# AO33/HiC_Genome_Assembler

Measured on AMD Instinct MI355X. Metric: Part1+Part2 wall-clock (s) and bins/s on N x N contact map, higher is better.
Workload: dtype f64

## Files before the change

### hic_genome_assembler_amd/_lib.py

```python
from __future__ import annotations

import ctypes
import os

import numpy as np

_HERE = os.path.dirname(os.path.abspath(__file__))
LIB_PATH = os.environ.get("HICMI_LIB") or os.path.join(_HERE, "libhicmi.so")
_lib = None

c_i64 = ctypes.c_int64
c_dbl = ctypes.c_double
_vp = ctypes.c_void_p
_M64 = (1 << 64) - 1

SIGNATURES = {
    "hicmi_abi_version": (ctypes.c_int, []),
    "hicmi_last_error": (ctypes.c_char_p, []),
    "hicmi_device_count": (ctypes.c_int, [ctypes.POINTER(ctypes.c_int)]),
    "hicmi_create": (ctypes.c_int, [ctypes.c_int, ctypes.POINTER(_vp)]),
    "hicmi_destroy": (ctypes.c_int, [_vp]),
    "hicmi_stream": (ctypes.c_int, [_vp, ctypes.POINTER(_vp)]),
    "hicmi_synchronize": (ctypes.c_int, [_vp]),
    "hicmi_set_contacts_host": (ctypes.c_int, [_vp, _vp, c_i64]),
    "hicmi_set_contacts_host_f32": (ctypes.c_int, [_vp, _vp, c_i64]),
    "hicmi_set_contacts_device": (ctypes.c_int, [_vp, _vp, c_i64, c_i64]),
    "hicmi_contacts_device": (ctypes.c_int, [_vp, ctypes.POINTER(_vp), ctypes.POINTER(c_i64), ctypes.POINTER(c_i64)]),
    "hicmi_load_hicpro_matrix": (ctypes.c_int, [ctypes.c_char_p, _vp, c_i64, _vp, ctypes.c_int, ctypes.POINTER(c_i64)]),
    "hicmi_row_sums": (ctypes.c_int, [_vp, _vp, _vp]),
    "hicmi_set_row_shard": (ctypes.c_int, [_vp, c_i64, c_i64]),
    "hicmi_set_row_sums": (ctypes.c_int, [_vp, _vp, _vp]),
    "hicmi_compact": (ctypes.c_int, [_vp, _vp, c_i64]),
    "hicmi_group_sums": (ctypes.c_int, [_vp, _vp, _vp, c_i64, c_i64, _vp, _vp]),
    "hicmi_upgma": (ctypes.c_int, [_vp, _vp, _vp]),
    "hicmi_rank_matrix": (ctypes.c_int, [_vp, _vp]),
    "hicmi_presort_state": (ctypes.c_int, [_vp, _vp, _vp]),
    "hicmi_get_rank_rows": (ctypes.c_int, [_vp, c_i64, c_i64, ctypes.c_int, _vp]),
    "hicmi_get_similarity_row": (ctypes.c_int, [_vp, c_i64, _vp]),
    "hicmi_cut_scan": (ctypes.c_int, [_vp, c_i64, c_i64, c_dbl, _vp, _vp]),
    "hicmi_filter_scan": (ctypes.c_int, [_vp, c_i64, c_i64, c_i64, c_i64, c_dbl, _vp, _vp]),
    "hicmi_first_pass_cuts": (ctypes.c_int, [_vp, c_i64, c_i64, c_dbl, _vp, c_i64, _vp, _vp, c_i64, _vp]),
    "hicmi_filter_cuts": (ctypes.c_int, [_vp, _vp, c_i64, c_dbl, _vp, c_i64, _vp, _vp]),
    "hicmi_first_pass_cuts_multi": (ctypes.c_int, [_vp, c_i64, _vp, _vp, c_dbl, _vp, c_i64, _vp, _vp, c_i64, _vp]),
    "hicmi_filter_cuts_multi": (ctypes.c_int, [_vp, c_i64, _vp, _vp, _vp, _vp, c_i64, _vp, _vp]),
    "hicmi_hypergeom_decide": (ctypes.c_int, [c_i64, c_i64, c_i64, c_i64, c_dbl]),
    "hicmi_hypergeom_sf": (c_dbl, [c_i64, c_i64, c_i64, c_i64]),
    "hicmi_selftest_division": (ctypes.c_int, [_vp, ctypes.c_uint64, c_i64, ctypes.POINTER(ctypes.c_uint64)]),
    "hicmi_label_linkage": (ctypes.c_int, [_vp, c_i64, _vp]),
    "hicmi_leaf_order": (ctypes.c_int, [_vp, c_i64, _vp]),
    "hicmi_get_raw_merges": (ctypes.c_int, [_vp, _vp]),
    "hicmi_nnchain_stats": (ctypes.c_int, [_vp, _vp]),
    "hicmi_p2_select": (ctypes.c_int, [_vp, _vp, c_i64]),
    "hicmi_p2_total": (ctypes.c_int, [_vp, ctypes.POINTER(c_dbl)]),
    "hicmi_p2_score": (ctypes.c_int, [_vp, _vp, c_i64, c_i64, c_dbl, _vp]),
    "hicmi_p2_score_exact": (ctypes.c_int, [_vp, _vp, c_i64, c_i64, c_dbl, _vp]),
    "hicmi_p2_layout": (ctypes.c_int, [_vp, _vp, _vp, c_i64]),
    "hicmi_p2_set_arrangement": (ctypes.c_int, [_vp, _vp, _vp, c_i64]),
    "hicmi_p2_arrangement_total": (ctypes.c_int, [_vp, ctypes.POINTER(c_dbl)]),
    "hicmi_p2_arrangement_score": (ctypes.c_int, [_vp, c_dbl, ctypes.POINTER(c_dbl)]),
    "hicmi_p2_score_insertions": (ctypes.c_int, [_vp, ctypes.c_int32, c_dbl, _vp]),
    "hicmi_p2_window_tables": (ctypes.c_int, [_vp, c_i64, _vp, c_i64, _vp, c_i64]),
    "hicmi_p2_score_window": (ctypes.c_int, [_vp, c_i64, c_i64, _vp]),
    "hicmi_p2_decide_window": (ctypes.c_int, [_vp, c_i64, c_i64, c_dbl, c_dbl, c_dbl, ctypes.POINTER(c_i64),
                                              ctypes.POINTER(c_dbl), ctypes.POINTER(c_dbl)]),
    "hicmi_p2_window_shortlist": (ctypes.c_int, [_vp, c_i64, c_i64, c_i64, c_dbl, c_dbl, c_dbl, c_i64, _vp, _vp, _vp]),
    "hicmi_p2_decide_insertion": (ctypes.c_int, [_vp, _vp, _vp, c_i64, ctypes.c_int32, ctypes.c_int32,
                                                 ctypes.POINTER(c_i64), ctypes.POINTER(ctypes.c_int32),
                                                 ctypes.POINTER(c_dbl)]),
    "hicmi_p2_insert_all": (ctypes.c_int, [_vp, _vp, _vp, c_i64, _vp, c_i64, ctypes.POINTER(c_dbl)]),
    "hicmi_scan_valid_pairs": (ctypes.c_int, [ctypes.c_char_p, ctypes.c_char_p, _vp, c_i64, _vp, _vp, c_i64, ctypes.c_int,
                                              ctypes.POINTER(c_i64), ctypes.POINTER(c_i64), ctypes.POINTER(_vp)]),
    "hicmi_scan_fetch": (ctypes.c_int, [_vp, _vp, _vp, _vp]),
    "hicmi_plot_percentiles": (ctypes.c_int, [_vp, ctypes.c_int, _vp, c_i64, _vp, c_i64, _vp]),
    "hicmi_plot_downsample": (ctypes.c_int, [_vp, ctypes.c_int, _vp, c_i64, c_i64, _vp]),
    "hicmi_p2_insert_all_multi": (ctypes.c_int, [c_i64, _vp, _vp, _vp, _vp, _vp, _vp, _vp]),
    "hicmi_p2_start_all": (ctypes.c_int, [c_i64] + [_vp] * 16),
    "hicmi_p2_scan_arranged": (ctypes.c_int, [_vp, _vp, _vp, c_i64, c_i64, _vp, c_i64, _vp, c_i64, ctypes.POINTER(c_dbl),
                                              ctypes.POINTER(c_dbl), ctypes.POINTER(c_i64)]),
    "hicmi_p2_support": (ctypes.c_int, [_vp, _vp, _vp, c_i64, c_dbl, _vp, _vp]),
    "hicmi_p2_support_multi": (ctypes.c_int, [c_i64, _vp, _vp, _vp, _vp, _vp, _vp, _vp]),
    "hicmi_p2_breaks": (ctypes.c_int, [_vp, _vp, _vp, c_i64, c_dbl, c_i64, _vp, _vp]),
    "hicmi_p2_breaks_multi": (ctypes.c_int, [c_i64, _vp, _vp, _vp, _vp, _vp, c_i64, _vp, _vp]),
    "hicmi_p2_scan_pass": (ctypes.c_int, [_vp, _vp, _vp, c_i64, c_i64, c_dbl, ctypes.POINTER(c_dbl), ctypes.POINTER(c_dbl),
                                          ctypes.POINTER(ctypes.c_int32)]),
    "hicmi_p2_scan_all": (ctypes.c_int, [_vp, _vp, _vp, c_i64, c_i64, c_dbl, ctypes.POINTER(c_dbl), ctypes.POINTER(c_dbl),
                          ctypes.POINTER(c_i64)]),
    "hicmi_hmm_load_obs": (ctypes.c_int, [_vp, _vp, c_i64, c_i64, c_i64]),
    "hicmi_hmm_set_obs": (ctypes.c_int, [_vp, _vp, c_i64, c_i64]),
    "hicmi_hmm_set_width": (ctypes.c_int, [_vp, c_i64]),
    "hicmi_hmm_get_obs": (ctypes.c_int, [_vp, c_i64, c_i64, _vp]),
    "hicmi_hmm_dist2": (ctypes.c_int, [_vp, _vp, c_i64, _vp]),
    "hicmi_hmm_col_stats": (ctypes.c_int, [_vp, _vp, _vp]),
    "hicmi_hmm_kmeans": (ctypes.c_int, [_vp, _vp, c_i64, c_dbl, _vp, _vp, ctypes.POINTER(c_dbl), ctypes.POINTER(c_i64)]),
    "hicmi_hmm_fit": (ctypes.c_int, [_vp, _vp, _vp, _vp, _vp, c_i64, c_dbl, _vp, ctypes.POINTER(c_i64)]),
    "hicmi_hmm_decode": (ctypes.c_int, [_vp, _vp, _vp, _vp, _vp, _vp]),
    "hicmi_hmm_load_obs_slot": (ctypes.c_int, [_vp, c_i64, _vp, c_i64, c_i64, c_i64]),
    "hicmi_hmm_use_obs": (ctypes.c_int, [_vp, c_i64]),
    "hicmi_hmm_dist2_multi": (ctypes.c_int, [_vp, c_i64, _vp, _vp, _vp, _vp, _vp]),
    "hicmi_hmm_kmeans_multi": (ctypes.c_int, [_vp, c_i64, _vp, _vp, _vp, _vp, _vp, _vp, _vp, _vp]),
    "hicmi_louvain_graph": (ctypes.c_int, [_vp, _vp, c_i64]),
    "hicmi_louvain_set_graph": (ctypes.c_int, [_vp, _vp, c_i64]),
    "hicmi_louvain_get_graph": (ctypes.c_int, [_vp, _vp, _vp, _vp]),
    "hicmi_louvain_level0": (ctypes.c_int, [_vp, c_i64, _vp, _vp, _vp, _vp, _vp, _vp]),
    "hicmi_louvain_induced": (ctypes.c_int, [_vp, _vp, c_i64, c_i64, _vp]),
    "hicmi_louvain_modularity": (ctypes.c_int, [_vp, _vp, c_i64, c_i64, _vp]),
    "hicmi_timing_reset": (ctypes.c_int, [_vp]),
    "hicmi_timing_enable": (ctypes.c_int, [_vp, ctypes.c_int]),
    "hicmi_timing_get": (ctypes.c_int, [_vp, ctypes.c_char_p, c_i64, _vp, _vp, _vp, c_i64, ctypes.POINTER(c_i64)]),
}


class HicmiError(RuntimeError):
    pass


def load():
    global _lib
    if _lib is not None:
        return _lib
    if not os.path.exists(LIB_PATH):
        raise HicmiError("libhicmi.so is not built (%s): run `make -C %s` - this package has no CPU fallback"
                         % (LIB_PATH, os.path.join(_HERE, "csrc")))
    try:
        import torch
    except ImportError:
        pass
    lib = ctypes.CDLL(LIB_PATH)
    for name, (res, args) in SIGNATURES.items():
        fn = getattr(lib, name)
        fn.restype = res
        fn.argtypes = args
    if lib.hicmi_abi_version() != 1:
        raise HicmiError("libhicmi ABI version mismatch")
    _lib = lib
    return lib


def _check(rc):
    if rc != 0:
        raise HicmiError("libhicmi error %d: %s" % (rc, load().hicmi_last_error().decode("utf-8", "replace")))


def _ptr(a):
    return None if a is None else a.ctypes.data_as(_vp)


def load_hicpro_matrix(path, bin_ids, threads: int = 0):
    ids = np.ascontiguousarray(bin_ids, dtype=np.int64)
    n = len(ids)
    out = np.empty((n, n), dtype=np.float64)
    edges = c_i64()
    _check(load().hicmi_load_hicpro_matrix(os.fsencode(path), _ptr(ids), n, _ptr(out), int(threads), ctypes.byref(edges)))
    return out, edges.value


def scan_valid_pairs(path, names, pairs, threads: int = 0):
    enc = [n.encode("utf-8") for n in names]
    blob = b"".join(enc)
    off = np.zeros(len(enc) + 1, np.int64)
    if enc:
        off[1:] = np.cumsum([len(e) for e in enc])
    pa = np.ascontiguousarray([p[0] for p in pairs], dtype=np.int32)
    pb = np.ascontiguousarray([p[1] for p in pairs], dtype=np.int32)
    n_hits, n_lines, handle = c_i64(), c_i64(), _vp()
    _check(load().hicmi_scan_valid_pairs(os.fsencode(path), blob, _ptr(off), len(enc), _ptr(pa), _ptr(pb), len(pa), int(threads),
                                         ctypes.byref(n_hits), ctypes.byref(n_lines), ctypes.byref(handle)))
    idx = np.empty(n_hits.value, np.int32)
    p1 = np.empty(n_hits.value, np.int64)
    p2 = np.empty(n_hits.value, np.int64)
    _check(load().hicmi_scan_fetch(handle, _ptr(idx), _ptr(p1), _ptr(p2)))
    return idx, p1, p2, n_lines.value


def hypergeom_sf(x, M, n, N) -> float:
    return float(load().hicmi_hypergeom_sf(int(x), int(M), int(n), int(N)))


def hypergeom_decide(x, M, n, N, psig) -> int:
    return int(load().hicmi_hypergeom_decide(int(x), int(M), int(n), int(N), float(psig)))


class Context:

    def __init__(self, device: int = 0):
        self._lib = load()
        h = _vp()
        _check(self._lib.hicmi_create(int(device), ctypes.byref(h)))
        self._h = h
        self.device = int(device)
        self.n = 0
        self._keepalive = None
        self._workers = []
        self._n_window_cand = 0
        self._lv_m = 0
        self.shard = (0, 1)

    def close(self):
        for w in getattr(self, "_workers", []):
            w.close()
        self._workers = []
        if getattr(self, "_h", None):
            self._lib.hicmi_destroy(self._h)
            self._h = None

    def workers(self, count: int):
        pool = getattr(self, "_workers", None)
        if pool is None:
            pool = self._workers = []
        ptr, n, ld = _vp(), c_i64(), c_i64()
        _check(self._lib.hicmi_contacts_device(self._h, ctypes.byref(ptr), ctypes.byref(n), ctypes.byref(ld)))
        while len(pool) < count:
            pool.append(Context(self.device))
        for w in pool[:count]:
            if getattr(w, "_shared_from", None) != (ptr.value, n.value, ld.value):
                w.set_contacts_device(ptr.value, n.value, ld.value, keepalive=self)
                w._shared_from = (ptr.value, n.value, ld.value)
        return pool[:count]

    def __del__(self):
        try:
            self.close()
        except Exception:
            pass

    def __enter__(self):
        return self

    def __exit__(self, *exc):
# ... 118 lines not shown

    def filter_cuts(self, cuts, psig):
        cuts = np.ascontiguousarray(cuts, dtype=np.int32)
        out = np.empty(self.n, np.int32)
        m, warned = c_i64(0), c_i64(0)
        _check(self._lib.hicmi_filter_cuts(self._h, _ptr(cuts), len(cuts), float(psig), _ptr(out), self.n,
                                           ctypes.byref(m), ctypes.byref(warned)))
        return [int(v) for v in out[:m.value]], int(warned.value)

    SCAN_MAX_SETS = 64

    def first_pass_cuts_multi(self, sets, psig):
        out = []
        n = self.n
        for c0 in range(0, len(sets), self.SCAN_MAX_SETS):
            part = sets[c0:c0 + self.SCAN_MAX_SETS]
            k = len(part)
            ms = np.array([int(a) for a, _b in part], np.int64)
            si = np.array([int(b) for _a, b in part], np.int64)
            cuts = np.empty((k, n), np.int32)
            mlog = np.empty((k, n, 2), np.int32)
            nc, nl = np.zeros(k, np.int64), np.zeros(k, np.int64)
            _check(self._lib.hicmi_first_pass_cuts_multi(self._h, k, _ptr(ms), _ptr(si), float(psig), _ptr(cuts), n,
                                                         _ptr(nc), _ptr(mlog), n, _ptr(nl)))
            out += [([int(v) for v in cuts[j, :nc[j]]], [(int(a), int(b)) for a, b in mlog[j, :nl[j]]]) for j in range(k)]
        return out

    def filter_cuts_multi(self, lists, psigs):
        out = []
        n = self.n
        for c0 in range(0, len(lists), self.SCAN_MAX_SETS):
            part = [np.asarray(v, dtype=np.int32) for v in lists[c0:c0 + self.SCAN_MAX_SETS]]
            k = len(part)
            off = np.zeros(k + 1, np.int64)
            off[1:] = np.cumsum([len(v) for v in part])
            cand = np.ascontiguousarray(np.concatenate(part) if off[-1] else np.zeros(1, np.int32), dtype=np.int32)
            ps = np.array([float(v) for v in psigs[c0:c0 + self.SCAN_MAX_SETS]], np.float64)
            kept = np.empty((k, n), np.int32)
            m, warned = np.zeros(k, np.int64), np.zeros(k, np.int64)
            _check(self._lib.hicmi_filter_cuts_multi(self._h, k, _ptr(off), _ptr(cand), _ptr(ps), _ptr(kept), n,
                                                     _ptr(m), _ptr(warned)))
            out += [([int(v) for v in kept[j, :m[j]]], int(warned[j])) for j in range(k)]
        return out

    def p2_select(self, sel):
        sel = np.ascontiguousarray(sel, dtype=np.int32)
        _check(self._lib.hicmi_p2_select(self._h, _ptr(sel), len(sel)))
        self._arr_sig = None

    def p2_total(self) -> float:
        t = c_dbl()
        _check(self._lib.hicmi_p2_total(self._h, ctypes.byref(t)))
        return t.value

    def p2_score(self, perms, total: float):
        perms = np.ascontiguousarray(perms, dtype=np.int32)
        if perms.ndim != 2:
            raise ValueError("perms must be (n_cand, n_used)")
        out = np.empty(perms.shape[0], np.float64)
        if perms.shape[0]:
            _check(self._lib.hicmi_p2_score(self._h, _ptr(perms), perms.shape[0], perms.shape[1], float(total), _ptr(out)))
        return out

    def p2_score_exact(self, perms, total: float):
        perms = np.ascontiguousarray(perms, dtype=np.int32)
        if perms.ndim != 2:
            raise ValueError("perms must be (n_cand, n_used)")
        out = np.empty(perms.shape[0], np.float64)
        if perms.shape[0]:
            _check(self._lib.hicmi_p2_score_exact(self._h, _ptr(perms), perms.shape[0], perms.shape[1], float(total),
                                                  _ptr(out)))
        return out

    def p2_layout(self, scaf_start, scaf_len):
        a = np.ascontiguousarray(scaf_start, dtype=np.int32)
        b = np.ascontiguousarray(scaf_len, dtype=np.int32)
        _check(self._lib.hicmi_p2_layout(self._h, _ptr(a), _ptr(b), len(a)))
        self._arr_sig = None

    def p2_set_arrangement(self, ids, rev):
        a = np.ascontiguousarray(ids, dtype=np.int32)
        b = np.ascontiguousarray(rev, dtype=np.uint8)
        sig = a.tobytes() + b.tobytes()
        if sig == getattr(self, "_arr_sig", None):
            return
        _check(self._lib.hicmi_p2_set_arrangement(self._h, _ptr(a), _ptr(b), len(a)))
        self._arr_len = len(a)
        self._arr_sig = sig

    def p2_arrangement_total(self) -> float:
        t = c_dbl()
        _check(self._lib.hicmi_p2_arrangement_total(self._h, ctypes.byref(t)))
        return t.value

    def p2_arrangement_score(self, total: float) -> float:
        t = c_dbl()
        _check(self._lib.hicmi_p2_arrangement_score(self._h, float(total), ctypes.byref(t)))
        return t.value

    def p2_score_insertions(self, new_id: int, total: float):
        out = np.empty(2 * (self._arr_len + 1), np.float64)
        _check(self._lib.hicmi_p2_score_insertions(self._h, int(new_id), float(total), _ptr(out)))
        return out

    def p2_window_tables(self, orders, orients):
        a = np.ascontiguousarray(orders, dtype=np.int8)
        b = np.ascontiguousarray(orients, dtype=np.uint8)
        _check(self._lib.hicmi_p2_window_tables(self._h, a.shape[1], _ptr(a), a.shape[0], _ptr(b), b.shape[0]))
        self._n_window_cand = a.shape[0] * b.shape[0]

    def p2_score_window(self, first: int, k: int):
        if not self._n_window_cand:
            raise HicmiError("p2_window_tables has not been called")
        out = np.empty(self._n_window_cand, np.float64)
        _check(self._lib.hicmi_p2_score_window(self._h, int(first), int(k), _ptr(out)))
        return out

    def p2_decide_window(self, first, k, total, floor, cur_fast):
        pick, best, pf = c_i64(), c_dbl(), c_dbl()
        _check(self._lib.hicmi_p2_decide_window(self._h, int(first), int(k), float(total), float(floor),
                                                float("nan") if cur_fast is None else float(cur_fast),
                                                ctypes.byref(pick), ctypes.byref(best), ctypes.byref(pf)))
        return pick.value, best.value, pf.value

    def p2_window_shortlist(self, first, count, k, total, floor, cur_fast=None, cap=4096):
        n_near = np.zeros(int(count), np.int64)
        idx = np.zeros((int(count), int(cap)), np.int64)
        fast = np.zeros((int(count), int(cap)), np.float64)
        _check(self._lib.hicmi_p2_window_shortlist(self._h, int(first), int(count), int(k), float(total), float(floor),
                                                   float("nan") if cur_fast is None else float(cur_fast), int(cap),
                                                   _ptr(n_near), _ptr(idx), _ptr(fast)))
        return [None if m > cap else (idx[w, :m].copy(), fast[w, :m].copy()) for w, m in enumerate(n_near.tolist())]

    def p2_decide_insertion(self, ids, rev, new_id, new_rev_now):
        a = np.ascontiguousarray(ids, dtype=np.int32)
        b = np.ascontiguousarray(rev, dtype=np.uint8)
        gap, r, best = c_i64(), ctypes.c_int32(), c_dbl()
        _check(self._lib.hicmi_p2_decide_insertion(self._h, _ptr(a), _ptr(b), len(a), int(new_id), int(new_rev_now),
                                                   ctypes.byref(gap), ctypes.byref(r), ctypes.byref(best)))
        self._arr_sig = a.tobytes() + b.tobytes()
        self._arr_len = len(a)
        return gap.value, r.value, best.value

    def p2_insert_all(self, ids, rev, new_ids):
        s0, k = len(ids), len(new_ids)
        a = np.zeros(s0 + k, np.int32); a[:s0] = ids
        b = np.zeros(s0 + k, np.uint8); b[:s0] = rev
        nw = np.ascontiguousarray(new_ids, dtype=np.int32)
        best = c_dbl()
        _check(self._lib.hicmi_p2_insert_all(self._h, _ptr(a), _ptr(b), s0, _ptr(nw), k, ctypes.byref(best)))
        self._arr_sig = None
        return a, b, best.value

    @staticmethod
    def p2_insert_all_multi(jobs):
        n = len(jobs)
        if n == 0:
            return []
        lib = jobs[0][0]._lib
        keep, a_l, b_l, nw_l = [], [], [], []
        for ctx, ids, rev, new_ids in jobs:
            s0, k = len(ids), len(new_ids)
            a = np.zeros(s0 + k, np.int32); a[:s0] = ids
            b = np.zeros(s0 + k, np.uint8); b[:s0] = rev
            a_l.append(a); b_l.append(b); nw_l.append(np.ascontiguousarray(new_ids, dtype=np.int32))
        handles = (ctypes.c_void_p * n)(*[j[0]._h for j in jobs])
        pa = (ctypes.c_void_p * n)(*[x.ctypes.data for x in a_l])
        pb = (ctypes.c_void_p * n)(*[x.ctypes.data for x in b_l])
        pn = (ctypes.c_void_p * n)(*[x.ctypes.data for x in nw_l])
        s0s = (c_i64 * n)(*[len(j[1]) for j in jobs])
        ks = (c_i64 * n)(*[len(j[3]) for j in jobs])
        best = (c_dbl * n)()
        _check(lib.hicmi_p2_insert_all_multi(n, handles, pa, pb, s0s, pn, ks, best))
        for ctx, _i, _r, _n in jobs:
            ctx._arr_sig = None
        return [(a_l[j], b_l[j], best[j]) for j in range(n)]

    @staticmethod
    def p2_start_all(jobs, tables):
        n = len(jobs)
        if n == 0:
            return []
        lib = jobs[0][0]._lib
        i32 = lambda col: np.ascontiguousarray(np.concatenate([np.asarray(j[col], dtype=np.int32) for j in jobs]), dtype=np.int32)
        sel, st, ln, ids = i32(1), i32(2), i32(3), i32(4)
        n_sel = (c_i64 * n)(*[len(j[1]) for j in jobs])
        n_scaf = (c_i64 * n)(*[len(j[2]) for j in jobs])
        ks = (c_i64 * n)(*[len(j[4]) for j in jobs])
        keep = {k: (np.ascontiguousarray(o, dtype=np.int8), np.ascontiguousarray(r, dtype=np.uint8)) for k, (o, r) in tables.items()}
        po = (ctypes.c_void_p * 9)(*[keep[k][0].ctypes.data if k in keep else None for k in range(9)])
        pr = (ctypes.c_void_p * 9)(*[keep[k][1].ctypes.data if k in keep else None for k in range(9)])
        no = (c_i64 * 9)(*[keep[k][0].shape[0] if k in keep else 0 for k in range(9)])
        nr = (c_i64 * 9)(*[keep[k][1].shape[0] if k in keep else 0 for k in range(9)])
        handles = (ctypes.c_void_p * n)(*[j[0]._h for j in jobs])
        total, pick, cost, status = (c_dbl * n)(), (c_i64 * n)(), (c_dbl * n)(), (ctypes.c_int32 * n)()
        _check(lib.hicmi_p2_start_all(n, handles, _ptr(sel), n_sel, _ptr(st), _ptr(ln), n_scaf, _ptr(ids), ks, po, no, pr, nr,
                                      total, pick, cost, status))
        for j, job in enumerate(jobs):
            ctx, k = job[0], len(job[4])
            ctx._arr_sig, ctx._arr_len = None, k
            if status[j] != 1:
                ctx._n_window_cand = keep[k][0].shape[0] * keep[k][1].shape[0]
        return [(total[j], int(pick[j]), cost[j], int(status[j])) for j in range(n)]

    def p2_scan_arranged(self, ids, rev, k, orders, orients, best):
        a = np.ascontiguousarray(ids, dtype=np.int32).copy()
        b = np.ascontiguousarray(rev, dtype=np.uint8).copy()
        o = np.ascontiguousarray(orders, dtype=np.int8)
        r = np.ascontiguousarray(orients, dtype=np.uint8)
        bst, total, rounds = c_dbl(float(best)), c_dbl(), c_i64()
        _check(self._lib.hicmi_p2_scan_arranged(self._h, _ptr(a), _ptr(b), len(a), int(k), _ptr(o), o.shape[0], _ptr(r), r.shape[0],
                                                ctypes.byref(total), ctypes.byref(bst), ctypes.byref(rounds)))
        self._arr_sig = None
        self._n_window_cand = o.shape[0] * r.shape[0]
        return a, b, bst.value, int(rounds.value), total.value

    def p2_support(self, ids, rev, total: float):
        a = np.ascontiguousarray(ids, dtype=np.int32)
        b = np.ascontiguousarray(rev, dtype=np.uint8)
        S = len(a)
        table, best = np.empty((S, S, 2), np.float64), np.empty((S, 2), np.int32)
        _check(self._lib.hicmi_p2_support(self._h, _ptr(a), _ptr(b), S, float(total), _ptr(table), _ptr(best)))
        self._arr_sig = a.tobytes() + b.tobytes()
        self._arr_len = S
        return table, best

    @staticmethod
    def p2_support_multi(jobs):
        n = len(jobs)
        if n == 0:
            return []
        lib = jobs[0][0]._lib
        a_l = [np.ascontiguousarray(j[1], dtype=np.int32) for j in jobs]
        b_l = [np.ascontiguousarray(j[2], dtype=np.uint8) for j in jobs]
        t_l = [np.empty((len(a), len(a), 2), np.float64) for a in a_l]
        o_l = [np.empty((len(a), 2), np.int32) for a in a_l]
        handles = (ctypes.c_void_p * n)(*[j[0]._h for j in jobs])
        pa, pb, pt, po = ((ctypes.c_void_p * n)(*[x.ctypes.data for x in arrs]) for arrs in (a_l, b_l, t_l, o_l))
        sizes = (c_i64 * n)(*[len(a) for a in a_l])
        totals = (c_dbl * n)(*[float(j[3]) for j in jobs])
        _check(lib.hicmi_p2_support_multi(n, handles, pa, pb, sizes, totals, pt, po))
        for (ctx, _i, _r, _t), a, b in zip(jobs, a_l, b_l):
            ctx._arr_sig = a.tobytes() + b.tobytes()
            ctx._arr_len = len(a)
        return list(zip(t_l, o_l))

    def p2_breaks(self, ids, rev, lengths, total: float, min_piece: int = 1):
        return Context.p2_breaks_multi([(self, ids, rev, lengths, total)], min_piece, single=True)[0]

    @staticmethod
    def p2_breaks_multi(jobs, min_piece: int = 1, single=False):
        n = len(jobs)
        if n == 0:
            return []
        lib = jobs[0][0]._lib
        a_l = [np.ascontiguousarray(j[1], dtype=np.int32) for j in jobs]
        b_l = [np.ascontiguousarray(j[2], dtype=np.uint8) for j in jobs]
        t_l = [np.empty((sum(max(int(ln) - 1, 0) for ln in j[3]), 8), np.float64) for j in jobs]
        o_l = [np.empty((len(a), 2), np.int32) for a in a_l]
        if single:
            _check(lib.hicmi_p2_breaks(jobs[0][0]._h, _ptr(a_l[0]), _ptr(b_l[0]), len(a_l[0]), float(jobs[0][4]), int(min_piece),
                                       t_l[0].ctypes.data, _ptr(o_l[0])))
        else:
            handles = (ctypes.c_void_p * n)(*[j[0]._h for j in jobs])
            pa, pb, pt, po = ((ctypes.c_void_p * n)(*[x.ctypes.data for x in arrs]) for arrs in (a_l, b_l, t_l, o_l))
            sizes = (c_i64 * n)(*[len(a) for a in a_l])
            totals = (c_dbl * n)(*[float(j[4]) for j in jobs])
            _check(lib.hicmi_p2_breaks_multi(n, handles, pa, pb, sizes, totals, int(min_piece), pt, po))
        for j, a, b in zip(jobs, a_l, b_l):
            j[0]._arr_sig = a.tobytes() + b.tobytes()
            j[0]._arr_len = len(a)
        return list(zip(t_l, o_l))

    def p2_scan_pass(self, ids, rev, k, total, best, cur_fast):
        a = np.ascontiguousarray(ids, dtype=np.int32).copy()
        b = np.ascontiguousarray(rev, dtype=np.uint8).copy()
        bst = c_dbl(float(best))
        cf = c_dbl(float("nan") if cur_fast is None else float(cur_fast))
        imp = ctypes.c_int32()
        _check(self._lib.hicmi_p2_scan_pass(self._h, _ptr(a), _ptr(b), len(a), int(k), float(total), ctypes.byref(bst),
                                            ctypes.byref(cf), ctypes.byref(imp)))
        self._arr_sig = None
        return a, b, bst.value, cf.value, bool(imp.value)

    def p2_scan_all(self, ids, rev, k, total, best, cur_fast):
        a = np.ascontiguousarray(ids, dtype=np.int32).copy()
        b = np.ascontiguousarray(rev, dtype=np.uint8).copy()
        bst = c_dbl(float(best))
        cf = c_dbl(float("nan") if cur_fast is None else float(cur_fast))
        rounds = c_i64()
        _check(self._lib.hicmi_p2_scan_all(self._h, _ptr(a), _ptr(b), len(a), int(k), float(total), ctypes.byref(bst),
                                           ctypes.byref(cf), ctypes.byref(rounds)))
        self._arr_sig = None
        return a, b, bst.value, cf.value, int(rounds.value)

    def plot_percentiles(self, kind, order, q):
        qa = np.ascontiguousarray(q, dtype=np.float64)
        out = np.empty(len(qa), np.float64)
        if order is None:
            n_sel, optr, keep = self.n, None, None
        else:
            keep = np.ascontiguousarray(order, dtype=np.int32)
            n_sel, optr = len(keep), _ptr(keep)
        _check(self._lib.hicmi_plot_percentiles(self._h, int(kind), optr, n_sel, _ptr(qa), len(qa), _ptr(out)))
        return out

# ... 232 lines not shown
```

### hic_genome_assembler_amd/csrc/api.hip

```cpp
#include <hip/hip_runtime.h>

#include <algorithm>
#include <cmath>
#include <cstdarg>
#include <climits>
#include <cstdio>
#include <cstdlib>
#include <cstring>
#include <numeric>
#include <string>
#include <unordered_map>
#include <functional>
#include <chrono>
#include <vector>

#include "../../include/hicmi.h"
#include "hicmi_internal.h"
#include "hyper.h"

using namespace hicmi;

static thread_local std::string g_err;

static int fail(int code, const char* fmt, ...)
{
    char buf[512];
    va_list ap;
    va_start(ap, fmt);
    vsnprintf(buf, sizeof(buf), fmt, ap);
    va_end(ap);
    g_err = buf;
    return code;
}

namespace hicmi { int set_error(int code, const char* msg) { return fail(code, "%s", msg); } }

#define HIPCHK(expr)                                                                              \
    do {                                                                                          \
        hipError_t _e = (expr);                                                                   \
        if (_e != hipSuccess) return fail(HICMI_EHIP, "%s: %s", #expr, hipGetErrorString(_e));     \
    } while (0)

enum Family { F_ROW_SUMS, F_BUILD_W, F_NNCHAIN, F_SORT, F_RANK_INVERT, F_CUT_COUNT, F_HYPER_FLAGS, F_P2_SELECT,
              F_P2_TOTAL, F_P2_SCORE, F_P2_EXACT, F_P2_INSERT, F_P2_WINDOW_G, F_P2_WINDOW_DELTA, F_PLOT, F_PRESORT, F_RANK_RELABEL,
              F_RANK_TIED, F_P2_WINDOW_FLOPS, F_COUNT };
static const char* kFamilyNames[F_COUNT] = {"row_sums", "build_w", "nnchain", "sort_rows", "rank_invert",
                                            "cut_count", "hyper_flags", "p2_select", "p2_total", "p2_score",
                                            "p2_score_exact", "p2_score_insert", "p2_window_G", "p2_window_delta", "plot",
                                            "presort_rows", "rank_relabel", "rank_rows_tied",
                                            "p2_window_G_flops"};

constexpr int kBaseSlabs = 256;

struct TimedRegion { int fam; hipEvent_t a, b; };

struct hicmi_ctx {
    int device = 0;
    hipStream_t stream = nullptr;
    int probed_xcc = 0;
    int64_t n = 0, ldc = 0;
    double* dC = nullptr;
    bool own_c = false;
    double *d_np = nullptr, *d_seq = nullptr;
    bool have_sums = false;
    int64_t shard_first = 0, shard_stride = 1;
    double *dW = nullptr, *dW2 = nullptr; int64_t ldw = 0; int64_t w_rows = 0;
    int *d_size = nullptr, *d_chain = nullptr, *d_status = nullptr;
    double* d_zraw = nullptr;
    std::vector<double> zraw;
    int32_t* d_order = nullptr;
    uint16_t *dR = nullptr, *dRank = nullptr; int64_t ldr = 0; int64_t r_rows = 0;
    void* d_sort_scratch = nullptr; size_t sort_scratch_cap = 0;
    bool have_rank = false;
    hipStream_t stream2 = nullptr; hipEvent_t ev_fork = nullptr, ev_join = nullptr;
    uint16_t* dRankS = nullptr; int64_t rank_s_rows = 0;
    int32_t* d_ident = nullptr; int64_t ident_cap = 0;
    unsigned char* d_ties = nullptr; int64_t ties_cap = 0;
    uint16_t* d_tie_bits = nullptr; int64_t tie_bits_rows = 0, ld_bits = 0;
    int32_t* d_row_list = nullptr; int64_t row_list_cap = 0;
    int64_t scan_first_batch = 0, scan_last_improved = 0;
    int64_t presort_tied_rows = 0;
    int presort_used = 0;
    int64_t presort_n = 0;
    bool presort_dealt = false;
    int32_t* d_x = nullptr; uint8_t* d_sig = nullptr; int64_t x_cap = 0;
    unsigned char* d_scan_multi = nullptr; size_t scan_multi_bytes = 0;
    int64_t cached_start = -1;
    double* d_tmp = nullptr; int64_t tmp_cap = 0;
    double* dM2 = nullptr; int64_t n2 = 0, ld2 = 0, m2_cap = 0;
    int32_t* d_sel = nullptr; int64_t sel_cap = 0;
    double* d_H = nullptr; int64_t h_cap = 0;
    int32_t* d_perms = nullptr; int64_t perms_cap = 0;
    double* d_scores = nullptr; int64_t scores_cap = 0;
    double* d_partial = nullptr; int64_t partial_cap = 0;
    double* d_T = nullptr; int64_t t_cap = 0;
    int32_t *d_scaf_start = nullptr, *d_scaf_len = nullptr; int64_t scaf_cap = 0, n_scaf = 0;
    std::vector<int32_t> h_scaf_start, h_scaf_len;
    int32_t* d_arr_packed = nullptr; int64_t arr_cap = 0;
    std::vector<int32_t> h_arr_packed;
    std::vector<int32_t> h_arr_id, h_arr_pos; std::vector<uint8_t> h_arr_rev;
    int32_t* d_pos2sel = nullptr; int64_t pos_cap = 0; int64_t n_arr = 0;
    int8_t* d_orders = nullptr; uint8_t* d_orients = nullptr; int64_t ord_cap = 0, ori_cap = 0;
    int tab_k = 0; int64_t n_orders = 0, n_orients = 0;
    std::vector<int8_t> h_orders; std::vector<uint8_t> h_orients;
    std::vector<int32_t> h_pos2sel;
    uint64_t arr_version = 0;
    uint64_t cur_lit_version = ~0ull; double cur_lit_total = 0.0, cur_lit_value = 0.0;
    double cache_total = 0.0; bool cache_valid = false;
    std::unordered_map<std::string, double> exact_cache;
    double* d_G = nullptr; int64_t g_cap = 0;
    double* d_delta = nullptr; int64_t delta_cap = 0;
    WindowBatchEntry* d_wb = nullptr; int64_t wb_cap = 0;
    int near_min_k = 7;
    unsigned char* d_wnear = nullptr; int64_t wnear_cap = 0;
    int32_t* d_arr_packed2 = nullptr; int64_t arr2_cap = 0;
    int32_t* d_pos2sel2 = nullptr; int64_t pos2_cap = 0;
    double* d_ins_T = nullptr; int64_t ins_t_cap = 0;
    double* d_ins_partial = nullptr; int64_t ins_partial_cap = 0;
    unsigned char* d_ins_blob = nullptr; int64_t ins_blob_cap = 0;
    InsStep* d_ins_steps = nullptr; int64_t ins_steps_cap = 0;
    SupRec* d_sup_recs = nullptr; int64_t sup_recs_cap = 0;
    BrkRec* d_brk_recs = nullptr; int64_t brk_recs_cap = 0;
    int32_t* d_gs_lists = nullptr; int64_t gs_lists_cap = 0;
    double* d_gs_sums = nullptr; int64_t gs_sums_cap = 0;
    struct HmmSlot { double* d_x = nullptr; int64_t cap = 0, T = 0, ld = 0, D = 0; };
    HmmSlot hslot[HICMI_HMM_MAX_SLOTS]; int hcur = 0;
    double* d_hx = nullptr; int64_t hmm_T = 0, hmm_ld = 0, hmm_D = 0;
    unsigned char* d_hmulti = nullptr; int64_t hmulti_cap = 0;
    int32_t* d_horder = nullptr; int64_t horder_cap = 0;
    double* d_hwork = nullptr; int64_t hwork_cap = 0;
    int32_t* d_hlab = nullptr; int64_t hlab_cap = 0;
    uint8_t* d_hbt = nullptr; int64_t hbt_cap = 0;
    double* d_hpart = nullptr; int64_t hpart_cap = 0;
    double* d_hsmall = nullptr; int64_t hsmall_cap = 0;
    double* d_hhist = nullptr; int64_t hhist_cap = 0;
    int* d_hst = nullptr; int64_t hst_cap = 0;
    double* d_lvA = nullptr; int64_t lvA_cap = 0; int64_t lv_m = 0;
    double* d_lvvec = nullptr; int64_t lvvec_cap = 0;
    int32_t* d_lvrows = nullptr; int64_t lvrows_cap = 0;
    unsigned char* d_lvwork = nullptr; int64_t lvwork_cap = 0;
    int32_t* d_plot_order = nullptr; int64_t plot_order_cap = 0;
    unsigned char* d_plot_work = nullptr; int64_t plot_work_cap = 0;
    double* d_plot_img = nullptr; int64_t plot_img_cap = 0;
    char* pin_up = nullptr; size_t pin_up_cap = 0, pin_up_off = 0;
    char* pin_down = nullptr; size_t pin_down_cap = 0;

    int timing = 0;
    std::vector<TimedRegion> regions;
    std::vector<hipEvent_t> pool;
    double ms[F_COUNT] = {0}; int64_t launches[F_COUNT] = {0}; double bytes[F_COUNT] = {0};
    double nn_scans = 0, nn_scan_cols = 0, nn_cache_hits = 0, nn_merges = 0; int64_t nn_retries = 0;
};

namespace {
hipError_t sync_stream(hicmi_ctx* c);

struct Timed {
    hicmi_ctx* c; int fam; hipEvent_t a = nullptr, b = nullptr; hipStream_t st;
    Timed(hicmi_ctx* ctx, int f, double algo_bytes, hipStream_t on_stream = nullptr) : c(ctx), fam(f), st(on_stream ? on_stream : ctx->stream)
    {
        c->launches[f]++; c->bytes[f] += algo_bytes;
        if (!on()) return;
        a = grab(); b = grab();
        hipEventRecord(a, st);
    }
    bool on() const { return c->timing == 1 || (c->timing == 2 && (fam <= F_RANK_INVERT || fam >= F_PRESORT)); }
    ~Timed()
    {
        if (!on()) return;
        hipEventRecord(b, st);
        c->regions.push_back({fam, a, b});
    }
    hipEvent_t grab()
    {
        if (!c->pool.empty()) { hipEvent_t e = c->pool.back(); c->pool.pop_back(); return e; }
        hipEvent_t e; hipEventCreate(&e); return e;
    }
};

int resolve_timing(hicmi_ctx* c)
{
    if (c->regions.empty()) return HICMI_OK;
    HIPCHK(sync_stream(c));
    if (c->stream2) HIPCHK(hipStreamSynchronize(c->stream2));
    for (auto& r : c->regions) {
        float ms = 0.f;
        if (hipEventElapsedTime(&ms, r.a, r.b) == hipSuccess) c->ms[r.fam] += ms;
        c->pool.push_back(r.a); c->pool.push_back(r.b);
    }
    c->regions.clear();
    return HICMI_OK;
}


hipError_t sync_stream(hicmi_ctx* c)
{
    hipError_t e = hipStreamSynchronize(c->stream);
    c->pin_up_off = 0;
    return e;
}

int upload(hicmi_ctx* c, void* dst, const void* src, size_t bytes)
{
    if (bytes == 0) return HICMI_OK;
    const size_t need = (bytes + 63) & ~(size_t)63;
    if (c->pin_up_off + need > c->pin_up_cap) {
        HIPCHK(sync_stream(c));
        if (need > c->pin_up_cap) {
            if (c->pin_up) (void)hipHostFree(c->pin_up);
            c->pin_up = nullptr; c->pin_up_cap = 0;
            size_t cap = std::max<size_t>(need * 2, (size_t)1 << 20);
            HIPCHK(hipHostMalloc((void**)&c->pin_up, cap, hipHostMallocDefault));
            c->pin_up_cap = cap;
        }
    }
    char* slot = c->pin_up + c->pin_up_off;
    memcpy(slot, src, bytes);
    c->pin_up_off += need;
    HIPCHK(hipMemcpyAsync(dst, slot, bytes, hipMemcpyHostToDevice, c->stream));
    return HICMI_OK;
}

int ensure_pin_down(hicmi_ctx* c, size_t bytes)
{
    if (bytes > c->pin_down_cap) {
        if (c->pin_down) (void)hipHostFree(c->pin_down);
        c->pin_down = nullptr; c->pin_down_cap = 0;
        size_t cap = std::max<size_t>(bytes * 2, (size_t)1 << 20);
        HIPCHK(hipHostMalloc((void**)&c->pin_down, cap, hipHostMallocDefault));
        c->pin_down_cap = cap;
    }
    return HICMI_OK;
}

int download(hicmi_ctx* c, void* dst, const void* src, size_t bytes)
{
    if (bytes == 0) { HIPCHK(sync_stream(c)); return HICMI_OK; }
    int rc_pin = ensure_pin_down(c, bytes);
    if (rc_pin) return rc_pin;
    HIPCHK(hipMemcpyAsync(c->pin_down, src, bytes, hipMemcpyDeviceToHost, c->stream));
    HIPCHK(sync_stream(c));
    memcpy(dst, c->pin_down, bytes);
    return HICMI_OK;
}

template <typename T>
int ensure(T*& p, int64_t& cap, int64_t need)
{
    if (need <= cap && p) return HICMI_OK;
    if (p) { (void)hipFree(p); p = nullptr; cap = 0; }
    if (need <= 0) need = 1;
    hipError_t e = hipMalloc((void**)&p, (size_t)need * sizeof(T));
    if (e != hipSuccess) { p = nullptr; return fail(HICMI_ENOMEM, "hipMalloc(%lld bytes): %s", (long long)(need * (int64_t)sizeof(T)), hipGetErrorString(e)); }
    cap = need;
    return HICMI_OK;
}

void free_dev(void* p) { if (p) (void)hipFree(p); }

void drop_matrix_state(hicmi_ctx* c)
{
    if (c->own_c) free_dev(c->dC);
    c->dC = nullptr; c->own_c = false; c->n = 0; c->ldc = 0;
    free_dev(c->d_np); free_dev(c->d_seq); c->d_np = c->d_seq = nullptr; c->have_sums = false;
    c->have_rank = false; c->cached_start = -1; c->n2 = 0;
    if (c->presort_n && c->stream2) (void)hipStreamSynchronize(c->stream2);
    c->presort_n = 0;
}

int alloc_sums(hicmi_ctx* c)
{
    HIPCHK(hipMalloc((void**)&c->d_np, sizeof(double) * (size_t)std::max<int64_t>(c->n, 1)));
    HIPCHK(hipMalloc((void**)&c->d_seq, sizeof(double) * (size_t)std::max<int64_t>(c->n, 1)));
// ... 1696 lines not shown
    int rc = window_near_enqueue(c, first0, count, k, total, floor, cur_fast, cap, p);
    if (rc) return rc;
    return window_near_collect(c, p, n_near, near, near_fast);
}

const int64_t kNearCap = 4096;

int check_window_call(hicmi_ctx* c, int64_t first, int64_t k)
{
    const int64_t S = (int64_t)c->h_arr_id.size();
    if (c->n_arr < 1 || S < 1) return fail(HICMI_EINVAL, "hicmi_p2_set_arrangement has not run");
    if (k != c->tab_k || c->h_orders.empty()) return fail(HICMI_EINVAL, "hicmi_p2_window_tables has not been called for k = %lld", (long long)k);
    if (first < 0 || first + k > S) return fail(HICMI_EINVAL, "window out of range");
    for (int64_t j = 0; j < k; j++) if (c->h_orders[(size_t)j] != j) return fail(HICMI_EINVAL, "orders[0] must be the identity");
    return HICMI_OK;
}
}

int hicmi_p2_decide_window(hicmi_ctx* c, int64_t first, int64_t k, double total, double floor, double cur_fast,
                           int64_t* pick_out, double* best_out, double* pick_fast_out)
{
    if (!c || !pick_out || !best_out || !pick_fast_out) return fail(HICMI_EINVAL, "NULL argument");
    int rc = check_window_call(c, first, k);
    if (rc) return rc;
    use_total(c, total);
    if (k >= c->near_min_k) {
        std::vector<int64_t> n_near; std::vector<std::vector<int64_t>> near; std::vector<std::vector<double>> near_fast;
        rc = window_near_batch(c, first, 1, k, total, floor, cur_fast, kNearCap, n_near, near, near_fast);
        if (rc) return rc;
        if (n_near[0] <= kNearCap)
            return decide_from_near(c, first, k, total, floor, cur_fast, window_c0(c, first, k), near[0], near_fast[0],
                                    pick_out, best_out, pick_fast_out);
    }
    std::vector<double> delta((size_t)(c->n_orders * c->n_orients));
    rc = window_batch(c, first, 1, k, delta.data());
    if (rc) return rc;
    return decide_from_delta(c, first, k, total, floor, cur_fast, delta.data(), pick_out, best_out, pick_fast_out);
}

int hicmi_p2_window_shortlist(hicmi_ctx* c, int64_t first, int64_t count, int64_t k, double total, double floor,
                              double cur_fast, int64_t cap, int64_t* n_near_out, int64_t* idx_out, double* fast_out)
{
    if (!c || !n_near_out || !idx_out || !fast_out || count < 1) return fail(HICMI_EINVAL, "bad arguments");
    int rc = check_window_call(c, first, k);
    if (rc) return rc;
    std::vector<int64_t> n_near; std::vector<std::vector<int64_t>> near; std::vector<std::vector<double>> near_fast;
    rc = window_near_batch(c, first, count, k, total, floor, cur_fast, cap, n_near, near, near_fast);
    if (rc) return rc;
    for (int64_t w = 0; w < count; w++) {
        n_near_out[w] = n_near[(size_t)w];
        for (size_t q = 0; q < near[(size_t)w].size(); q++) {
            idx_out[w * cap + (int64_t)q] = near[(size_t)w][q];
            fast_out[w * cap + (int64_t)q] = near_fast[(size_t)w][q];
        }
    }
    return HICMI_OK;
}

int hicmi_p2_decide_insertion(hicmi_ctx* c, const int32_t* ids, const uint8_t* rev, int64_t S, int32_t new_id,
                              int32_t new_rev_now, int64_t* gap_out, int32_t* rev_out, double* best_out)
{
    if (!c || !ids || !rev || !gap_out || !rev_out || !best_out || S < 1) return fail(HICMI_EINVAL, "bad arguments");
    if (c->n_scaf < 1) return fail(HICMI_EINVAL, "hicmi_p2_layout has not run");
    if (new_id < 0 || new_id >= c->n_scaf) return fail(HICMI_EINVAL, "new scaffold out of range");
    *gap_out = -1; *rev_out = 0; *best_out = 0.0;
    std::vector<int32_t> ids2(ids, ids + S); ids2.push_back(new_id);
    std::vector<uint8_t> rev2(rev, rev + S); rev2.push_back(new_rev_now ? 1 : 0);
    int rc = hicmi_p2_set_arrangement(c, ids2.data(), rev2.data(), S + 1);
    if (rc) return rc;
    double total = 0.0;
    rc = hicmi_p2_arrangement_total(c, &total);
    if (rc) return rc;
    use_total(c, total);
    rc = hicmi_p2_set_arrangement(c, ids, rev, S);
    if (rc) return rc;
    const int64_t gaps = S + 1;
    std::vector<double> by_gap_rev((size_t)(2 * gaps));
    rc = hicmi_p2_score_insertions(c, new_id, total, by_gap_rev.data());
    if (rc) return rc;
    std::vector<double> fast((size_t)(2 * gaps));
    std::vector<int32_t> tag_rev((size_t)(2 * gaps));
    int32_t o = new_rev_now ? 1 : 0;
    for (int64_t i = 0; i < gaps; i++) {
        tag_rev[(size_t)(2 * i)] = o; tag_rev[(size_t)(2 * i + 1)] = o ^ 1;
        fast[(size_t)(2 * i)] = by_gap_rev[(size_t)(2 * i + o)];
        fast[(size_t)(2 * i + 1)] = by_gap_rev[(size_t)(2 * i + (o ^ 1))];
        o ^= 1;
    }
    std::vector<int64_t> near;
    short_list(fast, 0.0, near);
    if (near.empty()) return HICMI_OK;
    const int32_t st = c->h_scaf_start[(size_t)new_id], ln = c->h_scaf_len[(size_t)new_id];
    std::vector<std::vector<int32_t>> rows(near.size());
    for (size_t q = 0; q < near.size(); q++) {
        const int64_t g = near[q] / 2;
        const int32_t r = tag_rev[(size_t)near[q]];
        const int P = c->h_arr_pos[(size_t)g];
        std::vector<int32_t>& row = rows[q];
        row.reserve((size_t)(c->n_arr + ln));
        row.insert(row.end(), c->h_pos2sel.begin(), c->h_pos2sel.begin() + P);
        if (r) for (int32_t e = 0; e < ln; e++) row.push_back(st + ln - 1 - e);
        else   for (int32_t e = 0; e < ln; e++) row.push_back(st + e);
        row.insert(row.end(), c->h_pos2sel.begin() + P, c->h_pos2sel.end());
    }
    std::vector<double> lit;
    rc = literal_scores(c, rows, total, lit);
    if (rc) return rc;
    double best = 0.0; int64_t pick = -1;
    for (size_t q = 0; q < near.size(); q++) if (lit[q] > best) { best = lit[q]; pick = near[q]; }
    if (pick >= 0) { *gap_out = pick / 2; *rev_out = tag_rev[(size_t)pick]; *best_out = best; }
    return HICMI_OK;
}


namespace {
void apply_insertion(int32_t* ids, uint8_t* rev, int64_t& S, int64_t gap, int32_t new_id, int32_t r)
{
    for (int64_t j = S; j > gap; j--) { ids[j] = ids[j - 1]; rev[j] = rev[j - 1]; }
    ids[gap] = new_id; rev[gap] = (uint8_t)(r ? 1 : 0);
    S++;
}

struct InsJob {
    hicmi_ctx* c; int32_t* ids; uint8_t* rev; int64_t S; const int32_t* new_ids; int64_t n_new;
    int64_t t = 0; double best = 0.0; bool device_ok = true;
};

int queue_insertions(hicmi_ctx* lead, const std::vector<InsJob*>& jobs)
{
    const int nj = (int)jobs.size();
    if (nj == 0) return HICMI_OK;
    const int NB = kBaseSlabs;
    static const int max_c = getenv("HICMI_P2_INS_MAXC") ? atoi(getenv("HICMI_P2_INS_MAXC")) : INS_MAXC;
    int64_t steps_max = 0;
    std::vector<size_t> blob_off((size_t)nj);
    size_t blob_bytes = 0;
    for (int j = 0; j < nj; j++) {
        InsJob& job = *jobs[(size_t)j];
        hicmi_ctx* c = job.c;
        int rc = hicmi_p2_set_arrangement(c, job.ids, job.rev, job.S);
        if (rc) return rc;
        if (c != lead) HIPCHK(sync_stream(c));
        const int64_t n_steps = job.n_new - job.t;
        int64_t n_max = c->n_arr;
        for (int64_t t = 0; t < n_steps; t++) n_max += c->h_scaf_len[(size_t)job.new_ids[job.t + t]];
        if (n_max * (int64_t)sizeof(int32_t) > 160 * 1024) return fail(HICMI_EUNSUPPORTED, "candidate longer than 40960 bins");
        const int64_t S_max = job.S + n_steps;
        rc = ensure(c->d_arr_packed2, c->arr2_cap, 3 * std::max<int64_t>(S_max, c->n_scaf) + 2);
        if (rc) return rc;
        rc = ensure(c->d_pos2sel2, c->pos2_cap, c->n2);
        if (rc) return rc;
        rc = ensure(c->d_ins_T, c->ins_t_cap, (1 + 2 * (int64_t)INS_MAXC) * n_max);
        if (rc) return rc;
        rc = ensure(c->d_ins_partial, c->ins_partial_cap, NB + n_max + 2 * (S_max + 1));
        if (rc) return rc;
        steps_max = std::max(steps_max, n_steps);
        blob_off[(size_t)j] = blob_bytes;
        blob_bytes += (sizeof(InsState) + sizeof(InsLog) * (size_t)n_steps + 15) & ~(size_t)15;
    }
    HIPCHK(hipSetDevice(lead->device));
    int rc = ensure(lead->d_ins_blob, lead->ins_blob_cap, (int64_t)blob_bytes);
    if (rc) return rc;
    rc = ensure(lead->d_ins_steps, lead->ins_steps_cap, steps_max * nj);
    if (rc) return rc;
    std::vector<InsStep> table((size_t)(steps_max * nj));
    std::vector<int> max_n_used((size_t)steps_max, 0), max_S((size_t)steps_max, 0), max_n_arr((size_t)steps_max, 0);
    double algo = 0.0;
    for (int j = 0; j < nj; j++) {
        InsJob& job = *jobs[(size_t)j];
        hicmi_ctx* c = job.c;
        const int64_t n_steps = job.n_new - job.t;
        int64_t n_max = c->n_arr;
        for (int64_t t = 0; t < n_steps; t++) n_max += c->h_scaf_len[(size_t)job.new_ids[job.t + t]];
        InsState* st = reinterpret_cast<InsState*>(lead->d_ins_blob + blob_off[(size_t)j]);
        InsLog* log = reinterpret_cast<InsLog*>(lead->d_ins_blob + blob_off[(size_t)j] + sizeof(InsState));
        int32_t* packed[2] = {c->d_arr_packed, c->d_arr_packed2};
        int32_t* pos2sel[2] = {c->d_pos2sel, c->d_pos2sel2};
        int64_t n_arr = c->n_arr;
        for (int64_t t = 0; t < steps_max; t++) {
            InsStep& d = table[(size_t)(t * nj + j)];
            memset(&d, 0, sizeof(d));
            d.st = st;
            if (t >= n_steps) continue;
            const int cur = (int)(t & 1), nxt = cur ^ 1;
            const int32_t nid = job.new_ids[job.t + t];
            const int L = c->h_scaf_len[(size_t)nid];
            d.M2 = c->dM2; d.H = c->d_H; d.ld2 = c->ld2;
            d.pos_cur = pos2sel[cur]; d.pos_nxt = pos2sel[nxt]; d.packed_cur = packed[cur]; d.packed_nxt = packed[nxt];
            d.T_total = c->d_ins_T; d.T_cand = c->d_ins_T + n_max; d.work = c->d_ins_T + (1 + (int64_t)INS_MAXC) * n_max;
            d.partial = c->d_ins_partial; d.log = log + t;
            d.n_arr = (int32_t)n_arr; d.S = (int32_t)(job.S + t); d.L = L; d.new_start = c->h_scaf_start[(size_t)nid];
            d.new_id = nid; d.active = 1; d.step = (int32_t)t; d.last = t == n_steps - 1;
            max_n_used[(size_t)t] = std::max(max_n_used[(size_t)t], (int)(n_arr + L));
            max_S[(size_t)t] = std::max(max_S[(size_t)t], d.S);
            max_n_arr[(size_t)t] = std::max(max_n_arr[(size_t)t], (int)n_arr);
            const double nn = (double)n_arr, Ld = (double)L, sd = (double)d.S;
            algo += 8.0 * (0.5 * nn * (nn - 1.0) + nn * nn + 2.0 * (sd + 1.0) * Ld * nn) + 4.0 * (nn + Ld) * (nn + Ld);
            n_arr += L;
        }
    }
    rc = upload(lead, lead->d_ins_steps, table.data(), sizeof(InsStep) * table.size());
    if (rc) return rc;
    {
        Timed timed(lead, F_P2_INSERT, algo);
        launch_insb_reset(lead->d_ins_steps, nj, lead->stream);
        for (int64_t t = 0; t < steps_max; t++) {
            const InsStep* st_t = lead->d_ins_steps + t * nj;
            const int nu = max_n_used[(size_t)t];
            launch_insb_fast(st_t, nj, max_S[(size_t)t], max_n_arr[(size_t)t], NB, lead->stream);
            launch_insb_shortlist(st_t, nj, max_S[(size_t)t], max_n_arr[(size_t)t], NB, kNearTop, max_c, lead->stream);
            launch_insb_diag_cand(st_t, nj, nu, lead->stream);
            launch_insb_cost(st_t, nj, nu, lead->stream);
            launch_insb_apply(st_t, nj, nu, lead->stream);
        }
    }
    HIPCHK(hipGetLastError());
    std::vector<unsigned char> blob(blob_bytes);
    rc = download(lead, blob.data(), lead->d_ins_blob, blob_bytes);
    if (rc) return rc;
    if (getenv("HICMI_PART2_PROFILE")) {
        int64_t hist[5] = {0, 0, 0, 0, 0}, all_direct = 0;
        for (int64_t t = 0; t < steps_max; t++) {
            int mx = -1, ran = 0;
            for (int j = 0; j < nj; j++) {
                if (t >= jobs[(size_t)j]->n_new - jobs[(size_t)j]->t) continue;
                const InsState* hs = reinterpret_cast<const InsState*>(blob.data() + blob_off[(size_t)j]);
                if (hs->fail >= 0 && t >= hs->fail) continue;
                const InsLog* hl = reinterpret_cast<const InsLog*>(blob.data() + blob_off[(size_t)j] + sizeof(InsState));
                const int ns = hl[t].n_short;
                hist[ns < 0 ? 0 : (ns > 3 ? 4 : ns + 1)]++;
                mx = std::max(mx, ns);
                ran++;
            }
            if (ran && mx < 0) all_direct++;
        }
        fprintf(stderr, "[hicmi] insertion short lists: direct %lld, literal with 0:%lld 1:%lld 2:%lld 3+:%lld candidates; "
                        "lock steps without any literal pass: %lld of %lld\n",
                (long long)hist[0], (long long)hist[1], (long long)hist[2], (long long)hist[3], (long long)hist[4],
                (long long)all_direct, (long long)steps_max);
    }
    for (int j = 0; j < nj; j++) {
        InsJob& job = *jobs[(size_t)j];
        const int64_t n_steps = job.n_new - job.t;
        const InsState* hst = reinterpret_cast<const InsState*>(blob.data() + blob_off[(size_t)j]);
        const InsLog* hlog = reinterpret_cast<const InsLog*>(blob.data() + blob_off[(size_t)j] + sizeof(InsState));
        const int64_t done = hst->fail >= 0 ? std::min<int64_t>(hst->fail, n_steps) : n_steps;
        for (int64_t t = 0; t < done; t++) {
            if (hlog[t].gap < 0 || hlog[t].gap > job.S) return fail(HICMI_ESTATE, "insertion log out of range");
            apply_insertion(job.ids, job.rev, job.S, hlog[t].gap, job.new_ids[job.t + t], hlog[t].rev);
            job.best = hlog[t].best;
        }
        job.t += done;
        hicmi_ctx* c = job.c;
        c->n_arr = 0; c->h_arr_id.clear(); c->h_arr_rev.clear(); c->h_arr_pos.clear(); c->h_pos2sel.clear();
    }
    return HICMI_OK;
}

int check_insert_job(const InsJob& job, int64_t S0)
{
    hicmi_ctx* c = job.c;
    if (!c || !job.ids || !job.rev || !job.new_ids || S0 < 1 || job.n_new < 1) return fail(HICMI_EINVAL, "bad arguments");
    if (c->n_scaf < 1) return fail(HICMI_EINVAL, "hicmi_p2_layout has not run");
    std::vector<uint8_t> used((size_t)c->n_scaf, 0);
    for (int64_t j = 0; j < S0 + job.n_new; j++) {
        const int32_t v = j < S0 ? job.ids[j] : job.new_ids[j - S0];
        if (v < 0 || v >= c->n_scaf || used[(size_t)v]) return fail(HICMI_EINVAL, "scaffolds must be distinct members of the layout");
        used[(size_t)v] = 1;
    }
    return HICMI_OK;
}

int host_insertion_step(InsJob& job)
{
    int64_t gap = -1; int32_t r = 0;
    int rc = hicmi_p2_decide_insertion(job.c, job.ids, job.rev, job.S, job.new_ids[job.t], 0, &gap, &r, &job.best);
    if (rc) return rc;
    if (gap < 0) { gap = 0; r = 0; job.best = 0.0; }
    apply_insertion(job.ids, job.rev, job.S, gap, job.new_ids[job.t], r);
    job.t++;
    return HICMI_OK;
}

int run_insert_jobs(std::vector<InsJob>& all)
{
    static const bool host_only = getenv("HICMI_P2_HOST_INSERT") != nullptr;
    for (InsJob& job : all) {
        int rc = check_insert_job(job, job.S);
        if (rc) return rc;
        if (job.S + job.n_new + 1 > 8192) job.device_ok = false;
    }
    while (true) {
        std::vector<InsJob*> todo;
        for (InsJob& job : all) if (job.t < job.n_new && job.device_ok && !host_only) todo.push_back(&job);
        if (!todo.empty()) {
            int rc = queue_insertions(todo[0]->c, todo);
            if (rc) return rc;
        }
        bool pending = false;
        for (InsJob& job : all) {
            if (job.t >= job.n_new) continue;
            do {
                int rc = host_insertion_step(job);
                if (rc) return rc;
            } while (job.t < job.n_new && (host_only || !job.device_ok));
            if (job.t < job.n_new) pending = true;
        }
        if (!pending) break;
    }
    return HICMI_OK;
}
}

int hicmi_p2_insert_all(hicmi_ctx* c, int32_t* ids, uint8_t* rev, int64_t S0, const int32_t* new_ids, int64_t n_new,
                        double* best_out)
{
    if (!c || !best_out) return fail(HICMI_EINVAL, "bad arguments");
    std::vector<InsJob> jobs(1);
    jobs[0].c = c; jobs[0].ids = ids; jobs[0].rev = rev; jobs[0].S = S0; jobs[0].new_ids = new_ids; jobs[0].n_new = n_new;
    int rc = run_insert_jobs(jobs);
    if (rc) return rc;
    *best_out = jobs[0].best;
    return HICMI_OK;
}

int hicmi_p2_insert_all_multi(int64_t n_jobs, hicmi_ctx* const* ctxs, int32_t* const* ids, uint8_t* const* rev,
                              const int64_t* S0, const int32_t* const* new_ids, const int64_t* n_new, double* best_out)
{
    if (n_jobs < 1 || !ctxs || !ids || !rev || !S0 || !new_ids || !n_new || !best_out) return fail(HICMI_EINVAL, "bad arguments");
    std::vector<InsJob> jobs((size_t)n_jobs);
    for (int64_t j = 0; j < n_jobs; j++) {
        InsJob& job = jobs[(size_t)j];
        job.c = ctxs[j]; job.ids = ids[j]; job.rev = rev[j]; job.S = S0[j]; job.new_ids = new_ids[j]; job.n_new = n_new[j];
        if (!job.c || job.c->device != ctxs[0]->device) return fail(HICMI_EINVAL, "contexts must share one device");
        for (int64_t q = 0; q < j; q++) if (ctxs[q] == ctxs[j]) return fail(HICMI_EINVAL, "one context per chromosome");
    }
    int rc = run_insert_jobs(jobs);
    if (rc) return rc;
    for (int64_t j = 0; j < n_jobs; j++) best_out[j] = jobs[(size_t)j].best;
    return HICMI_OK;
}

int hicmi_p2_support_multi(int64_t n_jobs, hicmi_ctx* const* ctxs, const int32_t* const* ids, const uint8_t* const* rev,
                           const int64_t* S, const double* totals, double* const* scores_out, int32_t* const* best_out)
{
    if (n_jobs < 1 || !ctxs || !ids || !rev || !S || !totals || !scores_out || !best_out) return fail(HICMI_EINVAL, "bad arguments");
    hicmi_ctx* lead = ctxs[0];
    const int NB = SUP_BASE_SLABS;
    std::vector<size_t> out_off((size_t)n_jobs, 0);
    std::vector<uint8_t> run((size_t)n_jobs, 0);
    size_t blob_bytes = 0;
    int64_t n_rec = 0;
    int max_S = 1, max_n = 1;
    for (int64_t j = 0; j < n_jobs; j++) {
        hicmi_ctx* c = ctxs[j];
        if (!c || !lead || c->device != lead->device) return fail(HICMI_EINVAL, "contexts must share one device");
        for (int64_t q = 0; q < j; q++) if (ctxs[q] == c) return fail(HICMI_EINVAL, "one context per chromosome");
        if (!ids[j] || !rev[j] || !scores_out[j] || !best_out[j] || S[j] < 1) return fail(HICMI_EINVAL, "bad arguments");
        if (S[j] > SUP_MAX_S) return fail(HICMI_EUNSUPPORTED, "more than %d scaffolds in one chromosome", SUP_MAX_S);
        int rc = hicmi_p2_set_arrangement(c, ids[j], rev[j], S[j]);
        if (rc) return rc;
        if (c != lead) HIPCHK(sync_stream(c));
        if (c->n_arr * (int64_t)sizeof(int32_t) > 160 * 1024) return fail(HICMI_EUNSUPPORTED, "candidate longer than 40960 bins");
        for (int64_t i = 0; i < 2 * S[j] * S[j]; i++) scores_out[j][i] = 0.0;
        for (int64_t i = 0; i < S[j]; i++) { best_out[j][2 * i] = -1; best_out[j][2 * i + 1] = 0; }
        if (c->n_arr < 2 || !(totals[j] > 0.0)) continue;
        run[(size_t)j] = 1;
        rc = ensure(c->d_ins_partial, c->ins_partial_cap, S[j] * (NB + c->n_arr + 2 * S[j]));
        if (rc) return rc;
        out_off[(size_t)j] = blob_bytes;
        blob_bytes += ((size_t)(2 * S[j] * S[j]) * sizeof(double) + (size_t)(2 * S[j]) * sizeof(int32_t) + 15) & ~(size_t)15;
        n_rec += S[j];
        max_S = std::max(max_S, (int)S[j]);
        max_n = std::max(max_n, (int)c->n_arr);
    }
    if (n_rec == 0) return HICMI_OK;
    HIPCHK(hipSetDevice(lead->device));
    int rc = ensure(lead->d_ins_blob, lead->ins_blob_cap, (int64_t)blob_bytes);
    if (rc) return rc;
    rc = ensure(lead->d_sup_recs, lead->sup_recs_cap, n_rec);
    if (rc) return rc;
    std::vector<SupRec> recs;
    recs.reserve((size_t)n_rec);
    double algo = 0.0;
    for (int64_t j = 0; j < n_jobs; j++) {
        if (!run[(size_t)j]) continue;
        hicmi_ctx* c = ctxs[j];
        const int64_t Sj = S[j], n = c->n_arr;
        double* d_scores = reinterpret_cast<double*>(lead->d_ins_blob + out_off[(size_t)j]);
        int32_t* d_best = reinterpret_cast<int32_t*>(d_scores + 2 * Sj * Sj);
        for (int64_t k = 0; k < Sj; k++) {
            SupRec d;
            memset(&d, 0, sizeof(d));
            const int32_t sid = ids[j][k];
            d.M2 = c->dM2; d.H = c->d_H; d.ld2 = c->ld2;
            d.pos = c->d_pos2sel; d.arr_pos = c->d_arr_packed + Sj;
            d.partial = c->d_ins_partial + k * (NB + n + 2 * Sj);
            d.scores = d_scores + 2 * Sj * k; d.best = d_best + 2 * k;
            d.total = totals[j];
            d.n = (int32_t)n; d.S = (int32_t)Sj; d.j = (int32_t)k;
            d.start = c->h_scaf_start[(size_t)sid]; d.L = c->h_scaf_len[(size_t)sid]; d.cur_rev = rev[j][k] ? 1 : 0;
            recs.push_back(d);
            const double nn = (double)(n - d.L);
            algo += 8.0 * (0.5 * nn * nn + nn * nn + 2.0 * (double)Sj * (double)d.L * nn);
        }
    }
    rc = upload(lead, lead->d_sup_recs, recs.data(), sizeof(SupRec) * recs.size());
    if (rc) return rc;
    {
        Timed timed(lead, F_P2_INSERT, algo);
        launch_sup(lead->d_sup_recs, (int)n_rec, max_S, max_n, kNearTop, lead->stream);
    }
    HIPCHK(hipGetLastError());
    std::vector<unsigned char> blob(blob_bytes);
    rc = download(lead, blob.data(), lead->d_ins_blob, blob_bytes);
    if (rc) return rc;
    for (int64_t j = 0; j < n_jobs; j++) {
        if (!run[(size_t)j]) continue;
        const size_t nd = (size_t)(2 * S[j] * S[j]);
        memcpy(scores_out[j], blob.data() + out_off[(size_t)j], nd * sizeof(double));
        memcpy(best_out[j], blob.data() + out_off[(size_t)j] + nd * sizeof(double), (size_t)(2 * S[j]) * sizeof(int32_t));
    }
    return HICMI_OK;
}

int hicmi_p2_support(hicmi_ctx* c, const int32_t* ids, const uint8_t* rev, int64_t S, double total, double* scores_out,
                     int32_t* best_out)
{
    return hicmi_p2_support_multi(1, &c, &ids, &rev, &S, &total, &scores_out, &best_out);
}

int hicmi_p2_breaks_multi(int64_t n_jobs, hicmi_ctx* const* ctxs, const int32_t* const* ids, const uint8_t* const* rev,
                          const int64_t* S, const double* totals, int64_t min_piece, double* const* scores_out,
                          int32_t* const* best_out)
{
    if (n_jobs < 1 || !ctxs || !ids || !rev || !S || !totals || !scores_out || !best_out || min_piece < 1)
        return fail(HICMI_EINVAL, "bad arguments");
    hicmi_ctx* lead = ctxs[0];
    const int NB = BRK_BASE_SLABS;
    std::vector<size_t> out_off((size_t)n_jobs, 0);
    std::vector<int64_t> n_scores((size_t)n_jobs, 0);
    std::vector<uint8_t> run((size_t)n_jobs, 0);
    size_t blob_bytes = 0;
    int64_t n_rec = 0;
    for (int64_t j = 0; j < n_jobs; j++) {
        hicmi_ctx* c = ctxs[j];
        if (!c || !lead || c->device != lead->device) return fail(HICMI_EINVAL, "contexts must share one device");
        for (int64_t q = 0; q < j; q++) if (ctxs[q] == c) return fail(HICMI_EINVAL, "one context per chromosome");
        if (!ids[j] || !rev[j] || !scores_out[j] || !best_out[j] || S[j] < 1) return fail(HICMI_EINVAL, "bad arguments");
        int rc = hicmi_p2_set_arrangement(c, ids[j], rev[j], S[j]);
        if (rc) return rc;
        if (c != lead) HIPCHK(sync_stream(c));
        if (c->n_arr * (int64_t)sizeof(int32_t) > 160 * 1024) return fail(HICMI_EUNSUPPORTED, "candidate longer than 40960 bins");
        int64_t cand = 0, scratch = NB, multi = 0;
        for (int64_t k = 0; k < S[j]; k++) {
            const int64_t L = c->h_scaf_len[(size_t)ids[j][k]];
            if (L < 2) continue;
            cand += 8 * (L - 1); scratch += L * L + 3 * (L - 1); multi++;
        }
        n_scores[(size_t)j] = cand;
        for (int64_t i = 0; i < cand; i++) scores_out[j][i] = 0.0;
        for (int64_t i = 0; i < S[j]; i++) { best_out[j][2 * i] = -1; best_out[j][2 * i + 1] = 0; }
        if (c->n_arr < 2 || !(totals[j] > 0.0) || multi == 0) continue;
        run[(size_t)j] = 1;
        rc = ensure(c->d_ins_partial, c->ins_partial_cap, scratch);
        if (rc) return rc;
        out_off[(size_t)j] = blob_bytes;
        blob_bytes += ((size_t)cand * sizeof(double) + (size_t)(2 * S[j]) * sizeof(int32_t) + 15) & ~(size_t)15;
        n_rec += multi;
    }
    if (n_rec == 0) return HICMI_OK;
    HIPCHK(hipSetDevice(lead->device));
    int rc = ensure(lead->d_ins_blob, lead->ins_blob_cap, (int64_t)blob_bytes);
    if (rc) return rc;
    rc = ensure(lead->d_brk_recs, lead->brk_recs_cap, n_rec);
// ... 1024 lines not shown
```

### hic_genome_assembler_amd/csrc/hicmi_internal.h

```cpp
#pragma once
#include <hip/hip_runtime.h>
#include <stdint.h>

#include <atomic>
#include <functional>

namespace hicmi {

inline void ensure_dynamic_lds(const void* func, std::atomic<int>& have, size_t bytes)
{
    if ((int)bytes > have.load(std::memory_order_relaxed)) {
        (void)hipFuncSetAttribute(func, hipFuncAttributeMaxDynamicSharedMemorySize, (int)bytes);
        have.store((int)bytes, std::memory_order_relaxed);
    }
}

static constexpr int SERIAL_BATCH = 16;

__device__ __forceinline__ double serial_sum_lds(const double* t, int from, int to, double acc)
{
    constexpr int B = SERIAL_BATCH;
    int i = from;
    if (i + B <= to) {
        double a[B];
// ... 111 lines not shown
                        int own_first, int own_step, hipStream_t s);

struct ScanState {
    int done;
    int mode;
    int start, cut, n_rows, recount;
    long long M;
    double psig;
    int min_size, stop_ind, loop_count, n_cuts, n_log, scans;
    int MD, n_alt, alt_off, f_i, f_keep_from, f_noise, f_round, f_max_rounds, f_warned;
    int pad;
    unsigned long long bytes;
};
static constexpr int SCAN_MAX_SETS = 64;
void launch_first_pass_multi_pairs(const uint16_t* rank, int64_t ldr, int n, int n_sets, ScanState* st, int32_t* x, uint8_t* sig,
                                   double psig0, int share, int32_t* cuts, int32_t* mlog, int log_cap, int pairs, hipStream_t s);
void launch_filter_multi_pairs(const uint16_t* rank, int64_t ldr, int n, int max_rows, int n_sets, ScanState* st, int32_t* x,
                               uint8_t* sig, double psig0, int share, int32_t* alt, uint8_t* filt, uint8_t* prev,
                               int32_t* seg, int32_t* seg_x, int pairs, hipStream_t s);

#if defined(__HIPCC__)
template <int M>
__device__ __forceinline__ uint32_t xor_lane(uint32_t v, int lane)
{
    if constexpr (M == 1) return (uint32_t)__builtin_amdgcn_mov_dpp((int)v, 0xB1, 0xf, 0xf, true);
    else if constexpr (M == 2) return (uint32_t)__builtin_amdgcn_mov_dpp((int)v, 0x4E, 0xf, 0xf, true);
    else if constexpr (M == 4) {
        const int t = __builtin_amdgcn_mov_dpp((int)v, 0x141, 0xf, 0xf, true);
        return (uint32_t)__builtin_amdgcn_mov_dpp(t, 0x1B, 0xf, 0xf, true);
    } else if constexpr (M == 8) {
        const int t = __builtin_amdgcn_mov_dpp((int)v, 0x140, 0xf, 0xf, true);
        return (uint32_t)__builtin_amdgcn_mov_dpp(t, 0x141, 0xf, 0xf, true);
    } else if constexpr (M == 16) {
        const auto r = __builtin_amdgcn_permlane16_swap(v, v, false, false);
        return (lane & 16) ? r[0] : r[1];
    } else {
        static_assert(M == 32, "xor_lane: M must be 1, 2, 4, 8, 16 or 32");
        const auto r = __builtin_amdgcn_permlane32_swap(v, v, false, false);
        return (lane & 32) ? r[0] : r[1];
    }
}
#endif

int  sort_padded_size(int n);
int  sort_workgroups(int n);
size_t sort_scratch_bytes(int n);
struct SortExtras {
    const int32_t* row_list = nullptr; int n_list = 0;
    uint8_t* tie_flag = nullptr; unsigned* tie_count = nullptr; unsigned tie_limit = 0;
    uint16_t* tie_bits = nullptr; int64_t ld_bits = 0;
    int max_workgroups = 0;
    int avoid_xcc = -1; unsigned* row_counter = nullptr;
};
static constexpr int GETREG_XCC_ID = 20 | (0 << 6) | (3 << 11);
int nnchain_local_xcc(const NNChainOptions& o, int n);
void launch_sort_rows(const double* C, int64_t ldc, const int32_t* order, const int32_t* inv, const double* np_sum,
                      const double* seq_sum, int n, void* scratch, uint16_t* R, int64_t ldr, int row_first, int row_stride,
                      hipStream_t s, const SortExtras& x = SortExtras());
void launch_rank_rows_tied(const uint16_t* R_storage, const uint16_t* tie_bits, int64_t ld_bits, const int32_t* order,
                           const int32_t* inv, int n, const int32_t* row_list, int n_list, uint16_t* rank, int64_t ldr,
                           hipStream_t s, int32_t* done = nullptr);
void launch_rank_relabel(const uint16_t* rank_storage, uint16_t* rank, int64_t ldr, int n, const int32_t* order, int row_first,
                         int row_stride, hipStream_t s);
size_t sort_radix_scratch_bytes(int n);
void launch_rank_rows_radix(const double* C, int64_t ldc, const int32_t* order, const int32_t* inv, const double* np_sum,
                            const double* seq_sum, int n, void* scratch, uint16_t* rank, int64_t ldr, int row_first,
                            int row_stride, hipStream_t s);
void launch_rank_invert(const uint16_t* R, uint16_t* rank, int64_t ldr, int n, int row_first, int row_stride, hipStream_t s,
                        const int32_t* row_list = nullptr, int n_list = 0);
void launch_similarity_row(const double* C, int64_t ldc, const int32_t* order, const double* np_sum,
                           const double* seq_sum, int n, int row, double* out, hipStream_t s);

void launch_p2_select(const double* C, int64_t ldc, const int32_t* sel, int n, double* M2, int64_t ld2, hipStream_t s);
void launch_p2_total(const double* M2, int64_t ld2, int n, double* T, double* total, hipStream_t s);
void launch_p2_score_exact(const double* M2, int64_t ld2, const int32_t* perms, int n_cand, int n_used, double total,
                           double* T, double* work, double* scores, hipStream_t s);
void launch_p2_score(const double* M2, int64_t ld2, const int32_t* perms, int n_cand, int n_used, const double* H,
                     double inv_total_unused, double total, double* scores, hipStream_t s);

void launch_p2_total_perm(const double* M2, int64_t ld2, const int32_t* d_perm, int n, double* T, double* total,
                          hipStream_t s);

struct WindowDesc {
    int32_t start[8];
    int32_t len[8];
    int32_t off[8];
    uint8_t rev[8];
};
void launch_arr_materialize(const int32_t* packed, int S, const int32_t* scaf_start, const int32_t* scaf_len, int n_arr,
                            int32_t* pos2sel, hipStream_t s);
void launch_p2_base_partial(const double* M2, int64_t ld2, const int32_t* pos2sel, int n_arr, const double* H, int n_tot,
                            int n_blocks, double* out, hipStream_t s);
void launch_p2_insert_delta(const double* M2, int64_t ld2, const int32_t* pos2sel, int n_arr, const int32_t* arr_pos,
                            int S, int new_start, int L, const double* H, int n_base_blocks, double* out, hipStream_t s);
struct WindowBatchEntry {
    WindowDesc w;
    int32_t p0, m;
    int64_t g_off;
    int32_t c0, pad;
};
void launch_p2_window_batch(const double* M2, int64_t ld2, const int32_t* pos2sel, int n, int k,
                            const WindowBatchEntry* wb, int n_win, int max_m, const int8_t* orders, const uint8_t* orients,
                            int n_ord, int n_ori, const double* H, double* G_all, double* delta_all, hipStream_t s);


int64_t window_table_doubles(int k);
void launch_p2_window_tables(const double* M2, int64_t ld2, const int32_t* pos2sel, int n, int k,
                             const WindowBatchEntry* wb, const WindowBatchEntry* h_wb, int n_win, int max_m, const int8_t* orders, const uint8_t* orients,
                             int n_ord, int n_ori, const double* H, double* tables, double* delta_all, hipStream_t s);
struct NearEntry { int32_t cand, pad; double fast; };
int window_near_blocks(int n_ord);
void launch_p2_window_near(const double* M2, int64_t ld2, const int32_t* pos2sel, int n, int k,
                           const WindowBatchEntry* wb, const WindowBatchEntry* h_wb, int n_win, int max_m, const int8_t* orders,
                           const uint8_t* orients, int n_ord, int n_ori, const double* H, double* tables, int whole, double total,
                           double cur_fast, double floor, double near_top, double* part, int32_t* count, NearEntry* near, int cap,
                           hipStream_t s);

__device__ __forceinline__ double wave_sum_s(double v)
{
#pragma unroll
    for (int off = 32; off >= 1; off >>= 1) v += __shfl_xor(v, off, 64);
    return v;
}

__device__ __forceinline__ double block_sum_256(double v, double* s_w)
{
    v = wave_sum_s(v);
    if ((threadIdx.x & 63) == 0) s_w[threadIdx.x >> 6] = v;
    __syncthreads();
    return (s_w[0] + s_w[1]) + (s_w[2] + s_w[3]);
}

__device__ __forceinline__ void base_partial_body(const double* __restrict__ M2, int64_t ld2, const int32_t* p, int n_arr,
                                                  const double* __restrict__ H, int n_tot, int blk, int n_blk,
                                                  double* __restrict__ out)
{
    __shared__ double s_w[4];
    const int lane = threadIdx.x & 63, wave = threadIdx.x >> 6;
    const double hn = H[n_tot - 1];
    double acc = 0.0;
    for (int a = blk * 4 + wave; a < n_arr - 1; a += n_blk * 4) {
        const double* __restrict__ row = M2 + (int64_t)p[a] * ld2;
#pragma unroll 4
        for (int b = a + 1 + lane; b < n_arr; b += 64) acc += row[p[b]] * (hn - H[b - a - 1]);
    }
    double sum = block_sum_256(acc, s_w);
    if (threadIdx.x == 0) out[0] = sum;
}

static constexpr int INS_MAXC = 8;
struct InsState {
    int32_t fail;
    int32_t n_short;
    int32_t direct, pad;
    int32_t gap[INS_MAXC], rev[INS_MAXC], idx[INS_MAXC];
    double total;
    double lit[INS_MAXC];
};
struct InsLog { int32_t gap, rev; double best; int32_t n_short, pad; };
struct InsStep {
    const double* M2; const double* H; int64_t ld2;
    const int32_t* pos_cur; int32_t* pos_nxt;
    const int32_t* packed_cur; int32_t* packed_nxt;
    double *T_total, *T_cand, *work, *partial;
    InsState* st; InsLog* log;
    int32_t n_arr, S, L, new_start, new_id, active, step, last;
};
void launch_insb_reset(const InsStep* steps, int n_chrom, hipStream_t s);
void launch_insb_fast(const InsStep* steps, int n_chrom, int max_S, int max_n_arr, int n_base_blocks, hipStream_t s);
void launch_insb_shortlist(const InsStep* steps, int n_chrom, int max_S, int max_n_arr, int n_base_blocks, double near_top,
                           int max_c, hipStream_t s);
void launch_insb_diag_cand(const InsStep* steps, int n_chrom, int max_n_used, hipStream_t s);
void launch_insb_cost(const InsStep* steps, int n_chrom, int max_n_used, hipStream_t s);
void launch_insb_apply(const InsStep* steps, int n_chrom, int max_n_used, hipStream_t s);

static constexpr int SUP_BASE_SLABS = 64;
static constexpr int SUP_MAX_S = 4096;
struct SupRec {
    const double* M2; const double* H; int64_t ld2;
    const int32_t* pos;
    const int32_t* arr_pos;
    double* partial;
    double* scores;
    int32_t* best;
    double total;
    int32_t n, S, j, start, L, cur_rev;
};
void launch_sup(const SupRec* recs, int n_rec, int max_S, int max_n, double near_top, hipStream_t s);

static constexpr int BRK_BASE_SLABS = 64;
struct BrkRec {
    const double* M2; const double* H; int64_t ld2;
    const int32_t* pos;
    double* X;
    double* pq;
    double* base;
    double* scores;
    int32_t* best;
    double total;
    int64_t wg0;
    int32_t n, B, L, min_piece;
    int32_t n_base, pad;
};
void launch_brk(const BrkRec* recs, int n_rec, int64_t n_wg, double near_top, hipStream_t s);

static constexpr int GS_CHUNK = 64;
struct GsChunk { int32_t row0, cnt, group, pad; };
void launch_group_sums(const double* C, int64_t ld, int n, int G, int S, const int32_t* rows, const GsChunk* chunks,
                       int n_chunks, const int32_t* group_chunk0, const int32_t* scaf, const int32_t* sbins,
                       const int32_t* soff, double* partial, double* binsum, double* scafsum, bool plain, hipStream_t s);

void launch_plot_select(const double* C, int64_t ldc, const double* np_sum, const double* seq_sum, int kind,
                        const int32_t* order, int n_sel, int n_targets, struct SelectState* d_state, unsigned int* d_hist,
                        hipStream_t s);
size_t plot_select_state_bytes();
size_t plot_select_hist_bytes();
int plot_select_max_targets();
void plot_select_fill(void* host_state, const unsigned long long* ranks, int n_targets);
double plot_select_value(const void* host_state, int t);
void launch_plot_downsample(const double* C, int64_t ldc, const double* np_sum, const double* seq_sum, int kind,
                            const int32_t* order, int n_sel, int px, double* out, hipStream_t s);

enum { HMM_P_MEAN = 0, HMM_P_VAR = 2, HMM_P_MOV = 4, HMM_P_IV = 6, HMM_P_LOGV = 8, HMM_P_MU2V = 10, HMM_P_SCALARS = 12 };
enum { HMM_S_CONST = 0, HMM_S_A = 2, HMM_S_LOGA = 6, HMM_S_PI = 10, HMM_S_LOGPI = 12, HMM_S_XI = 14, HMM_S_POST = 18,
       HMM_S_COUNT = 32 };
int  hmm_col_chunks(int T, int D);
__host__ __device__ inline void hmm_col_shape(int T, int R, int& rows_per, int& Rr)
{
    rows_per = (T + R - 1) / R;
    Rr = (T + rows_per - 1) / rows_per;
}
struct HmmKmProb {
    const double* X; int64_t ld; int T, D;
    int nc, rows_per, Rr, max_iter;
    int64_t rows[2];
    double tol;
    double *cen, *sums, *part, *out;
    int32_t* lab;
};
enum { HMM_KM_LLOYD = 0, HMM_KM_FINAL = 1, HMM_KM_SUM = 2, HMM_KM_DONE = 3 };
struct HmmKmState { int phase, cur, it, strict, changed, n1; double inertia; };
void launch_hmm_obs(const double* C, int64_t ldc, const int32_t* order, const double* np_sum, const double* seq_sum,
                    int c, int T, int D, double* X, hipStream_t s);
void launch_hmm_colsum(int mode, const double* X, int64_t ld, int T, int D, const double* shift, const int32_t* labels,
                       const double* g, double* part, double* out, hipStream_t s);
void launch_hmm_dist2(const double* X, int64_t ld, int T, int D, const double* cen, int nc, double* dist, hipStream_t s);
void launch_hmm_assign(const double* X, int64_t ld, int T, int D, const double* cen, const int32_t* old_labels,
                       int32_t* labels, double* mind, int* st, hipStream_t s);
void launch_hmm_center_update(const double* sums, int T, int D, const int* st, double* cen, double* shift_out, hipStream_t s);
void launch_hmm_sum(const double* v, int n, double* out, hipStream_t s);
void launch_hmm_params(const double* sums, int D, int from_sums, double* P, hipStream_t s);
void launch_hmm_emission(const double* X, int64_t ld, int T, int D, const double* P, double* L, hipStream_t s);
void launch_hmm_fb(const double* L, int T, double* P, int D, double* alpha, double* beta, double* gam, double* hist, int it,
                   hipStream_t s);
void launch_hmm_viterbi(const double* L, int T, const double* P, int D, uint8_t* bt, int32_t* states, hipStream_t s);
void launch_hmm_multi_seed(const HmmKmProb* pr, HmmKmState* st, int n_prob, int max_rows, int kmeans, hipStream_t s);
void launch_hmm_dist2_multi(const HmmKmProb* pr, int n_prob, int max_T, hipStream_t s);
void launch_hmm_kmeans_multi_step(const HmmKmProb* pr, HmmKmState* st, int* done, int n_prob, int max_T, int max_items,
                                  int max_2d, hipStream_t s);

static constexpr int LOUVAIN_MAX_M = 16384;
static constexpr int LOUVAIN_MAX_ROUNDS = 1024;
__host__ __device__ inline size_t louvain_round_bytes(int m) { return (size_t)m * (4 * sizeof(double) + 8 * sizeof(int)); }
int  louvain_level0_lds_max();
void launch_louvain_graph(const double* C, int64_t ldc, const int32_t* rows, const double* np_sum, const double* seq_sum, int m,
                          double* A, hipStream_t s);
void launch_louvain_status(const double* A, int m, double* diag, double* rowsum, double* chunk, double* dsum, double* gdeg,
                           double* total, hipStream_t s);
void launch_louvain_level0(const double* A, int m, const double* gdeg, const double* loops, const double* total, int rounds,
                           const uint64_t* st_in, int32_t* n2c_out, uint64_t* st_out, int32_t* info, double* deg_out,
                           double* int_out, unsigned char* scratch, hipStream_t s);
void launch_louvain_induced(const double* A, int m, const int32_t* members, const int32_t* moff, int k, double* rowagg,
                            double* B, hipStream_t s);
void launch_louvain_score(const double* A, int m, const int32_t* parts, int rounds, const double* gdeg, const double* total,
                          double* same, double* acc, double* q, hipStream_t s);

}
```

### hic_genome_assembler_amd/csrc/k_part2.hip

```cpp
#include <cstdlib>

#include "hicmi_internal.h"

namespace hicmi {

__global__ __launch_bounds__(256) void k_p2_select(const double* __restrict__ C, int64_t ldc,
                                                   const int32_t* __restrict__ sel, int n, double* __restrict__ M2,
                                                   int64_t ld2)
{
    int r = blockIdx.y;
    int c = blockIdx.x * 256 + threadIdx.x;
    if (c >= n) return;
    M2[(int64_t)r * ld2 + c] = C[(int64_t)sel[r] * ldc + sel[c]];
}

void launch_p2_select(const double* C, int64_t ldc, const int32_t* sel, int n, double* M2, int64_t ld2, hipStream_t s)
{
    hipLaunchKernelGGL(k_p2_select, dim3((n + 255) / 256, n), dim3(256), 0, s, C, ldc, sel, n, M2, ld2);
}

__device__ __forceinline__ double wave_sum(double v)
{
#pragma unroll
    for (int off = 32; off >= 1; off >>= 1) v += __shfl_xor(v, off, 64);
// ... 37 lines not shown
            const int l = l0 + slot;
            double r = 0.0;
            int o = 0, n = 0, lim = 0;
            if (l < nl) { o = leaf_off[l]; n = leaf_len[l]; lim = n - (n % 8); }
            {
                int64_t idx[16];
                double vals[16];
#pragma unroll
                for (int q = 0; q < 16; q++) {
                    const bool ok = l < nl && n >= 8 && q * 8 < lim;
                    const int t = o + q * 8 + k;
                    const int a = ok ? m.at(t) : 0, b = ok ? m.at(t + off) : 0;
                    idx[q] = (int64_t)a * ld2 + b;
                }
#pragma unroll
                for (int q = 0; q < 16; q++) vals[q] = (l < nl && n >= 8 && q * 8 < lim) ? M2[idx[q]] : 0.0;
                r = vals[0];
#pragma unroll
                for (int q = 1; q < 16; q++) if (q * 8 < lim) r += vals[q];
            }
            double s1 = r + __shfl_down(r, 1, 64);
            double s2 = s1 + __shfl_down(s1, 2, 64);
            double s3 = s2 + __shfl_down(s2, 4, 64);
            if (l < nl && k == 0) {
                double res;
                if (n < 8) { res = 0.0; for (int i = 0; i < n; i++) res += elem(o + i); }
                else { res = s3; for (int i = lim; i < n; i++) res += elem(o + i); }
                leaf_sum[l] = res;
            }
        }
        __syncthreads();
        if (lane == 0) acc += combine_leaves(nl, leaf_sum, leaf_dep, st_v, st_a);
    }
    return acc;
}

__device__ __forceinline__ double diag_sum_sequential(const double* __restrict__ M2, int64_t ld2, const IndexMap& m, int n_used,
                                                      int off)
{
    __shared__ double seq_buf[1024];
    const int lane = threadIdx.x, len = n_used - off;
    double acc = 0.0;
    for (int c0 = 0; c0 < len; c0 += 1024) {
        const int cnt = len - c0 < 1024 ? len - c0 : 1024;
        __syncthreads();
        for (int e = lane; e < cnt; e += 64) seq_buf[e] = M2[(int64_t)m.at(c0 + e) * ld2 + m.at(c0 + e + off)];
        __syncthreads();
        if (lane == 0) acc = serial_sum_lds(seq_buf, 0, cnt, acc);
    }
    return acc;
}

static bool numba_trace_order()
{
    const char* v = getenv("HICMI_P2_TRACE_ORDER");
    return v && (v[0] == 'n' || v[0] == 'N') && (v[1] == 'u' || v[1] == 'U') && (v[2] == 'm' || v[2] == 'M') && (v[3] == 'b' || v[3] == 'B');
}

__global__ __launch_bounds__(64) void k_p2_diag_sums(const double* __restrict__ M2, int64_t ld2,
                                                     const int32_t* __restrict__ perms, int n_used,
                                                     double* __restrict__ T, int sequential)
{
    const int cand = blockIdx.y, off = diag_of_block(blockIdx.x);
    if (off >= n_used) return;
    const IndexMap m = {perms ? perms + (int64_t)cand * n_used : nullptr, kNoSplice, 0, 0, 0};
    const double acc = sequential ? diag_sum_sequential(M2, ld2, m, n_used, off) : diag_sum_body(M2, ld2, m, n_used, off);
    if (threadIdx.x == 0) T[(int64_t)cand * n_used + off] = acc;
}

static constexpr int SERIAL_LDS_MAX = 8192;

__global__ __launch_bounds__(256) void k_p2_total_exact(const double* __restrict__ T, int n_used, double* __restrict__ total)
{
    extern __shared__ __attribute__((aligned(16))) unsigned char smem_t[];
    double* t = reinterpret_cast<double*>(smem_t);
    const bool staged = n_used <= SERIAL_LDS_MAX;
    if (staged) {
        for (int i = threadIdx.x; i < n_used; i += 256) t[i] = T[i];
        __syncthreads();
    }
    if (threadIdx.x != 0) return;
    double acc = 0.0;
    if (staged) acc = serial_sum_lds(t, 1, n_used, 0.0);
    else {
        for (int i = 1; i < n_used; i++) acc += T[i];
    }
    total[0] = acc;
}

__device__ __forceinline__ void cost_exact_body(const double* __restrict__ tg, int n_used, double total,
                                                double* __restrict__ wg, double* __restrict__ score_out)
{
    extern __shared__ __attribute__((aligned(16))) unsigned char smem_c[];
    const bool staged = n_used <= SERIAL_LDS_MAX;
    double* w = staged ? reinterpret_cast<double*>(smem_c) : wg;
    if (staged) {
        for (int i = threadIdx.x; i < n_used; i += 256) w[i] = tg[i];
        __syncthreads();
    }
    if (threadIdx.x == 0) {
        double cum = 0.0;
        if (staged) serial_prefix_lds(w, 1, n_used, 0.0);
        else {
            for (int i = 1; i < n_used; i++) { cum += tg[i]; w[i] = cum; }
        }
    }
    __syncthreads();
    for (int i = 1 + threadIdx.x; i < n_used; i += 256) w[i] = w[i] / total / (double)i;
    __syncthreads();
    if (threadIdx.x == 0) {
        double cost = 0.0;
        if (staged) cost = serial_sum_lds(w, 1, n_used, 0.0);
        else for (int i = 1; i < n_used; i++) cost += w[i];
        score_out[0] = cost;
    }
}

__global__ __launch_bounds__(256) void k_p2_cost_exact(const double* __restrict__ T, int n_used, double total,
                                                       double* __restrict__ work, double* __restrict__ scores)
{
    const int cand = blockIdx.x;
    cost_exact_body(T + (int64_t)cand * n_used, n_used, total, work + (int64_t)cand * n_used, scores + cand);
}

static std::atomic<int> g_lds_total{0}, g_lds_cost{0}, g_lds_score{0}, g_lds_insb_cost{0};

static size_t serial_lds_bytes(int n) { return n <= SERIAL_LDS_MAX ? (((size_t)n * sizeof(double)) + 15) & ~(size_t)15 : 16; }

void launch_p2_total(const double* M2, int64_t ld2, int n, double* T, double* total, hipStream_t s)
{
    if (n > 1) hipLaunchKernelGGL(k_p2_diag_sums, dim3(diag_grid(n), 1), dim3(64), 0, s, M2, ld2, (const int32_t*)nullptr, n, T, 0);
    ensure_dynamic_lds(reinterpret_cast<const void*>(k_p2_total_exact), g_lds_total, 65536);
    hipLaunchKernelGGL(k_p2_total_exact, dim3(1), dim3(256), serial_lds_bytes(n), s, T, n, total);
}

void launch_p2_total_perm(const double* M2, int64_t ld2, const int32_t* d_perm, int n, double* T, double* total,
                          hipStream_t s)
{
    if (n > 1) hipLaunchKernelGGL(k_p2_diag_sums, dim3(diag_grid(n), 1), dim3(64), 0, s, M2, ld2, d_perm, n, T, 0);
    ensure_dynamic_lds(reinterpret_cast<const void*>(k_p2_total_exact), g_lds_total, 65536);
    hipLaunchKernelGGL(k_p2_total_exact, dim3(1), dim3(256), serial_lds_bytes(n), s, T, n, total);
}

void launch_p2_score_exact(const double* M2, int64_t ld2, const int32_t* perms, int n_cand, int n_used, double total,
                           double* T, double* work, double* scores, hipStream_t s)
{
    if (n_cand <= 0) return;
    if (n_used > 1) hipLaunchKernelGGL(k_p2_diag_sums, dim3(diag_grid(n_used), n_cand), dim3(64), 0, s, M2, ld2, perms, n_used, T,
                                       numba_trace_order() ? 1 : 0);
    ensure_dynamic_lds(reinterpret_cast<const void*>(k_p2_cost_exact), g_lds_cost, 65536);
    hipLaunchKernelGGL(k_p2_cost_exact, dim3(n_cand), dim3(256), serial_lds_bytes(n_used), s, T, n_used, total, work, scores);
}

__global__ __launch_bounds__(64) void k_insb_diag_cand(const InsStep* __restrict__ steps, int sequential)
{
    const InsStep& d = steps[blockIdx.y];
    if (!d.active || d.st->fail >= 0) return;
    const int ns = d.st->n_short;
    if (ns == 0) return;
    const int n_used = d.n_arr + d.L, off = diag_of_block(blockIdx.x);
    if (off >= n_used) return;
    {
        const IndexMap m = {d.pos_cur, d.n_arr, 0x3fffffff, d.new_start, 0};
        const double acc = diag_sum_body(d.M2, d.ld2, m, n_used, off);
        if (threadIdx.x == 0) d.T_total[off] = acc;
    }
    for (int q = 0; q < ns; q++) {
        const IndexMap m = {d.pos_cur, d.packed_cur[d.S + d.st->gap[q]], d.L, d.new_start, d.st->rev[q]};
        const double acc = sequential ? diag_sum_sequential(d.M2, d.ld2, m, n_used, off) : diag_sum_body(d.M2, d.ld2, m, n_used, off);
        if (threadIdx.x == 0) d.T_cand[(int64_t)q * n_used + off] = acc;
    }
}

__global__ __launch_bounds__(256) void k_insb_cost(const InsStep* __restrict__ steps)
{
    extern __shared__ __attribute__((aligned(16))) unsigned char smem_ic[];
    __shared__ double s_total;
    const InsStep& d = steps[blockIdx.y];
    if (!d.active || d.st->fail >= 0) return;
    const int cand = blockIdx.x;
    if (cand >= d.st->n_short) return;
    const int n_used = d.n_arr + d.L;
    {
        double* t = reinterpret_cast<double*>(smem_ic);
        const bool staged = n_used <= SERIAL_LDS_MAX;
        if (staged) {
            for (int i = threadIdx.x; i < n_used; i += 256) t[i] = d.T_total[i];
            __syncthreads();
        }
        if (threadIdx.x == 0) {
            double acc = 0.0;
            if (staged) acc = serial_sum_lds(t, 1, n_used, 0.0);
            else for (int i = 1; i < n_used; i++) acc += d.T_total[i];
            s_total = acc;
            if (cand == 0) d.st->total = acc;
        }
        __syncthreads();
    }
    cost_exact_body(d.T_cand + (int64_t)cand * n_used, n_used, s_total, d.work + (int64_t)cand * n_used, d.st->lit + cand);
}

void launch_insb_diag_cand(const InsStep* steps, int n_chrom, int max_n_used, hipStream_t s)
{
    if (max_n_used < 2) return;
    hipLaunchKernelGGL(k_insb_diag_cand, dim3(diag_grid(max_n_used), n_chrom), dim3(64), 0, s, steps, numba_trace_order() ? 1 : 0);
}

void launch_insb_cost(const InsStep* steps, int n_chrom, int max_n_used, hipStream_t s)
{
    ensure_dynamic_lds(reinterpret_cast<const void*>(k_insb_cost), g_lds_insb_cost, 65536);
    const int max_staged = max_n_used < SERIAL_LDS_MAX ? max_n_used : SERIAL_LDS_MAX;
    hipLaunchKernelGGL(k_insb_cost, dim3(INS_MAXC, n_chrom), dim3(256), serial_lds_bytes(max_staged), s, steps);
}

__global__ __launch_bounds__(256) void k_p2_score(const double* __restrict__ M2, int64_t ld2,
                                                  const int32_t* __restrict__ perms, int n_used,
                                                  const double* __restrict__ H, double total,
                                                  double* __restrict__ scores)
{
    extern __shared__ __attribute__((aligned(16))) unsigned char smem[];
    int32_t* p = reinterpret_cast<int32_t*>(smem);
    __shared__ double s_w[4];
    const int cand = blockIdx.x, tid = threadIdx.x, lane = tid & 63, wave = tid >> 6;
    const int32_t* __restrict__ src = perms + (int64_t)cand * n_used;
    for (int i = tid; i < n_used; i += 256) p[i] = src[i];
    __syncthreads();
    const double hn = H[n_used - 1];
    double acc = 0.0;
    for (int a = wave; a < n_used - 1; a += 4) {
        const double* __restrict__ row = M2 + (int64_t)p[a] * ld2;
        for (int b = a + 1 + lane; b < n_used; b += 64) acc += row[p[b]] * (hn - H[b - a - 1]);
    }
    acc = wave_sum(acc);
    if (lane == 0) s_w[wave] = acc;
    __syncthreads();
    if (tid == 0) scores[cand] = ((s_w[0] + s_w[1]) + (s_w[2] + s_w[3])) / total;
}

void launch_p2_score(const double* M2, int64_t ld2, const int32_t* perms, int n_cand, int n_used, const double* H,
                     double, double total, double* scores, hipStream_t s)
{
    if (n_cand <= 0) return;
    size_t lds = (((size_t)n_used * sizeof(int32_t)) + 15) & ~(size_t)15;
    ensure_dynamic_lds(reinterpret_cast<const void*>(k_p2_score), g_lds_score, lds);
    hipLaunchKernelGGL(k_p2_score, dim3(n_cand), dim3(256), lds, s, M2, ld2, perms, n_used, H, total, scores);
}

}
```

### hic_genome_assembler_amd/csrc/k_part2_insert.hip

```cpp
#include "hicmi_internal.h"

namespace hicmi {

__global__ void k_insb_reset(const InsStep* __restrict__ steps)
{
    InsState* st = steps[blockIdx.x].st;
    if (threadIdx.x == 0 && steps[blockIdx.x].active) { st->fail = -1; st->n_short = 0; st->direct = 0; }
}

void launch_insb_reset(const InsStep* steps, int n_chrom, hipStream_t s)
{
    hipLaunchKernelGGL(k_insb_reset, dim3(n_chrom), dim3(64), 0, s, steps);
}

static constexpr int SL_THREADS = 256;
static constexpr int SL_LIST = 64;
static constexpr int SL_STAGE_MAX = 8192;

__global__ __launch_bounds__(SL_THREADS) void k_insb_shortlist(const InsStep* __restrict__ steps, int n_base_blocks,
                                                               double near_top, int max_c)
{
    extern __shared__ __attribute__((aligned(16))) unsigned char smem_sl[];
    double* buf = reinterpret_cast<double*>(smem_sl);
    __shared__ double s_base, s_wmax[SL_THREADS / 64];
    __shared__ int s_any[SL_THREADS / 64], s_cnt, s_list[SL_LIST];
    const InsStep& d = steps[blockIdx.x];
    InsState* st = d.st;
    const int tid = threadIdx.x;
    if (!d.active || st->fail >= 0) return;
    const int S = d.S, n_arr = d.n_arr;
    const double* __restrict__ partial = d.partial;
    const int32_t* __restrict__ arr_pos = d.packed_cur + S;
    double* part = buf + S + 1;
    const bool staged = n_arr <= SL_STAGE_MAX;
    const int n_stage = n_base_blocks + (staged ? n_arr : 0);
    for (int i = tid; i < n_stage; i += SL_THREADS) part[i] = partial[i];
    if (tid == 0) s_cnt = 0;
    __syncthreads();
    for (int g = tid; g < S; g += SL_THREADS) {
        const int P0 = arr_pos[g], P1 = arr_pos[g + 1];
        double acc = 0.0;
        if (staged) for (int u = P0; u < P1; u++) acc += part[n_base_blocks + u];
        else for (int u = P0; u < P1; u++) acc += partial[n_base_blocks + u];
        buf[g + 1] = acc;
    }
    __syncthreads();
    if (tid == 0) {
        s_base = serial_sum_lds(part, 0, n_base_blocks, 0.0);
        buf[0] = 0.0;
        serial_prefix_lds(buf, 1, S + 1, 0.0);
    }
    __syncthreads();
    const double base = s_base;
    const double* __restrict__ cross = partial + n_base_blocks + n_arr;
    const int n_cand = 2 * (S + 1);
    auto fast_of = [&](int i) -> double {
        const int g = i >> 1, first = g & 1;
        const int r = (i & 1) ? (first ^ 1) : first;
        return base - buf[g] + cross[2 * g + r];
    };
    double mx = -__builtin_inf();
    int any = 0;
    for (int i = tid; i < n_cand; i += SL_THREADS) {
        const double v = fast_of(i);
        if (isfinite(v)) { any = 1; if (v > mx) mx = v; }
    }
#pragma unroll
    for (int off = 32; off >= 1; off >>= 1) {
        const double o = __shfl_xor(mx, off, 64);
        const int oa = __shfl_xor(any, off, 64);
        if (o > mx) mx = o;
        any |= oa;
    }
    if ((tid & 63) == 0) { s_wmax[tid >> 6] = mx; s_any[tid >> 6] = any; }
    __syncthreads();
    double top = 0.0;
    int have = 0;
    for (int w = 0; w < SL_THREADS / 64; w++) { if (s_wmax[w] > top) top = s_wmax[w]; have |= s_any[w]; }
    if (!have) {
        if (tid == 0) { st->n_short = 0; st->direct = 0; }
        return;
    }
    const double thr = top - fabs(top) * near_top;
    for (int i = tid; i < n_cand; i += SL_THREADS) {
        const double v = fast_of(i);
        if (isfinite(v) && v >= thr) {
            const int slot = atomicAdd(&s_cnt, 1);
            if (slot < SL_LIST) s_list[slot] = i;
        }
    }
    __syncthreads();
    if (tid == 0) {
        int cnt = s_cnt;
        st->direct = 0;
        if (cnt > max_c && !(d.L == 1 && cnt <= 2 * max_c && cnt <= SL_LIST)) { st->fail = d.step; st->n_short = 0; return; }
        for (int a = 1; a < cnt; a++) {
            const int v = s_list[a];
            int b = a - 1;
            while (b >= 0 && s_list[b] > v) { s_list[b + 1] = s_list[b]; b--; }
            s_list[b + 1] = v;
        }
        if (d.L == 1) {
            int w = 0;
            for (int q = 0; q < cnt; q++) {
                const int i = s_list[q];
                if ((i & 1) && w > 0 && s_list[w - 1] == i - 1) continue;
                s_list[w++] = i;
            }
            cnt = w;
            if (cnt > max_c) { st->fail = d.step; st->n_short = 0; return; }
        }
        for (int q = 0; q < cnt; q++) {
            const int i = s_list[q], g = i >> 1, first = g & 1;
            st->idx[q] = i; st->gap[q] = g; st->rev[q] = (i & 1) ? (first ^ 1) : first;
        }
        if (cnt == 1 && !d.last && top > 0.0) { st->direct = 1; st->n_short = 0; }
        else st->n_short = cnt;
    }
}

static std::atomic<int> g_lds_shortlist{0};

void launch_insb_shortlist(const InsStep* steps, int n_chrom, int max_S, int max_n_arr, int n_base_blocks, double near_top,
                           int max_c, hipStream_t s)
{
    const int need = (max_S + 1) + n_base_blocks + (max_n_arr < SL_STAGE_MAX ? max_n_arr : SL_STAGE_MAX);
    const size_t lds = (((size_t)need * sizeof(double)) + 15) & ~(size_t)15;
    ensure_dynamic_lds(reinterpret_cast<const void*>(k_insb_shortlist), g_lds_shortlist, lds);
    hipLaunchKernelGGL(k_insb_shortlist, dim3(n_chrom), dim3(SL_THREADS), lds, s, steps, n_base_blocks, near_top,
                       max_c < 1 ? 1 : (max_c > INS_MAXC ? INS_MAXC : max_c));
}

__global__ __launch_bounds__(256) void k_insb_apply(const InsStep* __restrict__ steps)
{
    const InsStep& d = steps[blockIdx.y];
    const InsState* __restrict__ st = d.st;
    if (!d.active || st->fail >= 0) return;
    const int n_arr = d.n_arr, S = d.S, L = d.L, n_new = n_arr + L;
    if ((int)blockIdx.x * 256 >= n_new && blockIdx.x != 0) return;
    double best = 0.0;
    int pick = -1;
    const int ns = st->n_short, direct = st->direct;
    for (int q = 0; q < ns; q++) if (st->lit[q] > best) { best = st->lit[q]; pick = q; }
    if (direct) { pick = 0; best = __builtin_nan(""); }
    const int gap = pick >= 0 ? st->gap[pick] : 0, rev = pick >= 0 ? st->rev[pick] : 0;
    const int32_t* __restrict__ id_in = d.packed_cur;
    const int32_t* __restrict__ pos_in = d.packed_cur + S;
    const int32_t* __restrict__ rev_in = d.packed_cur + 2 * S + 1;
    const int P = pos_in[gap];
    const int pos = blockIdx.x * 256 + threadIdx.x;
    if (pos < n_new) {
        int v;
        if (pos < P) v = d.pos_cur[pos];
        else if (pos < P + L) v = d.new_start + (rev ? L - 1 - (pos - P) : pos - P);
        else v = d.pos_cur[pos - L];
        d.pos_nxt[pos] = v;
    }
    if (blockIdx.x == 0) {
        const int S1 = S + 1;
        int32_t* __restrict__ id_out = d.packed_nxt;
        int32_t* __restrict__ pos_out = d.packed_nxt + S1;
        int32_t* __restrict__ rev_out = d.packed_nxt + 2 * S1 + 1;
        for (int j = threadIdx.x; j < S1; j += 256) {
            id_out[j] = j < gap ? id_in[j] : (j == gap ? d.new_id : id_in[j - 1]);
            rev_out[j] = j < gap ? rev_in[j] : (j == gap ? rev : rev_in[j - 1]);
        }
        for (int j = threadIdx.x; j <= S1; j += 256) pos_out[j] = j <= gap ? pos_in[j] : pos_in[j - 1] + L;
        if (threadIdx.x == 0) { d.log->gap = gap; d.log->rev = rev; d.log->best = pick >= 0 ? best : 0.0; d.log->n_short = direct ? -1 : ns; }
    }
}

void launch_insb_apply(const InsStep* steps, int n_chrom, int max_n_used, hipStream_t s)
{
    hipLaunchKernelGGL(k_insb_apply, dim3((max_n_used + 255) / 256, n_chrom), dim3(256), 0, s, steps);
}

}
```

### hic_genome_assembler_amd/csrc/k_part2_search.hip

```cpp
#include "hicmi_internal.h"

namespace hicmi {

__device__ __forceinline__ double block_sum_1024(double v, double* s_w)
{
    v = wave_sum_s(v);
    if ((threadIdx.x & 63) == 0) s_w[threadIdx.x >> 6] = v;
    __syncthreads();
    double acc = 0.0;
#pragma unroll
    for (int i = 0; i < 16; i++) acc += s_w[i];
    return acc;
}

static size_t perm_lds_bytes(int n) { return (((size_t)n * sizeof(int32_t)) + 15) & ~(size_t)15; }

__global__ __launch_bounds__(256) void k_arr_materialize(const int32_t* __restrict__ packed, int S,
                                                         const int32_t* __restrict__ scaf_start,
                                                         const int32_t* __restrict__ scaf_len, int n_arr,
                                                         int32_t* __restrict__ pos2sel)
{
    const int32_t* __restrict__ arr_id = packed;
    const int32_t* __restrict__ arr_pos = packed + S;
    const int32_t* __restrict__ arr_rev = packed + 2 * S + 1;
    int q = blockIdx.x * 256 + threadIdx.x;
    if (q >= n_arr) return;
    int lo = 0, hi = S;
    while (hi - lo > 1) {
        int mid = (lo + hi) >> 1;
        if (arr_pos[mid] <= q) lo = mid; else hi = mid;
    }
    int sc = arr_id[lo], off = q - arr_pos[lo], len = scaf_len[sc];
    pos2sel[q] = scaf_start[sc] + (arr_rev[lo] ? len - 1 - off : off);
}

void launch_arr_materialize(const int32_t* packed, int S, const int32_t* scaf_start, const int32_t* scaf_len, int n_arr,
                            int32_t* pos2sel, hipStream_t s)
{
    if (n_arr <= 0) return;
    hipLaunchKernelGGL(k_arr_materialize, dim3((n_arr + 255) / 256), dim3(256), 0, s, packed, S, scaf_start, scaf_len,
                       n_arr, pos2sel);
}

__global__ __launch_bounds__(256) void k_p2_base_partial(const double* __restrict__ M2, int64_t ld2,
                                                         const int32_t* __restrict__ pos2sel, int n_arr,
                                                         const double* __restrict__ H, int n_tot,
                                                         double* __restrict__ partial)
{
    extern __shared__ __attribute__((aligned(16))) unsigned char smem[];
    int32_t* p = reinterpret_cast<int32_t*>(smem);
    for (int q = threadIdx.x; q < n_arr; q += 256) p[q] = pos2sel[q];
    __syncthreads();
    base_partial_body(M2, ld2, p, n_arr, H, n_tot, blockIdx.x, gridDim.x, partial + blockIdx.x);
}

static std::atomic<int> g_lds_base{0}, g_lds_straddle{0}, g_lds_cross{0}, g_lds_wdelta{0}, g_lds_wdelta1{0}, g_lds_wdelta_blk{0}, g_lds_wG{0}, g_lds_insb_base{0}, g_lds_insb_fast{0};

void launch_p2_base_partial(const double* M2, int64_t ld2, const int32_t* pos2sel, int n_arr, const double* H, int n_tot,
                            int n_blocks, double* out, hipStream_t s)
{
    ensure_dynamic_lds(reinterpret_cast<const void*>(k_p2_base_partial), g_lds_base, perm_lds_bytes(n_arr));
    hipLaunchKernelGGL(k_p2_base_partial, dim3(n_blocks), dim3(256), perm_lds_bytes(n_arr), s, M2, ld2, pos2sel, n_arr, H,
                       n_tot, out);
}

__device__ __forceinline__ void straddle_body(const double* __restrict__ M2, int64_t ld2, const int32_t* p, int n_arr,
                                              const int32_t* __restrict__ arr_pos, int g, int L,
                                              const double* __restrict__ H, double* s_w, double* __restrict__ out)
{
    const int lane = threadIdx.x & 63, wave = threadIdx.x >> 6;
    const int P0 = arr_pos[g], P1 = arr_pos[g + 1];
    const int len = P1 - P0, n_out = n_arr - len;
    double acc = 0.0;
    for (int u = P0 + wave; u < P1; u += 16) {
        const double* __restrict__ row = M2 + (int64_t)p[u] * ld2;
#pragma unroll 8
        for (int qq = lane; qq < n_out; qq += 64) {
            const bool before = qq < P0;
            const int pos = before ? qq : qq + len;
            const int d = before ? u - pos : pos - u;
            const double w = H[d + L - 1] - H[d - 1];
            const double v = row[p[pos]] * w;
            acc += before ? -v : v;
        }
    }
    double sum = block_sum_1024(acc, s_w);
    if (threadIdx.x == 0) out[0] = sum;
}

__device__ __forceinline__ void cross_body(const double* __restrict__ M2, int64_t ld2, const int32_t* p, int n_arr,
                                           const int32_t* __restrict__ arr_pos, int g, int r, int new_start, int L,
                                           const double* __restrict__ H, double* s_w, double* __restrict__ out)
{
    const int lane = threadIdx.x & 63, wave = threadIdx.x >> 6;
    const int P = arr_pos[g];
    const double hn = H[n_arr + L - 1];
    double acc = 0.0;
    for (int e = wave; e < L; e += 16) {
        const int xe = new_start + (r ? L - 1 - e : e);
        const double* __restrict__ row = M2 + (int64_t)xe * ld2;
#pragma unroll 4
        for (int q = lane; q < n_arr; q += 64) {
            int d = q < P ? (P + e - q) : (q + L - (P + e));
            acc += row[p[q]] * (hn - H[d - 1]);
        }
        for (int e2 = e + 1 + lane; e2 < L; e2 += 64) {
            int x2 = new_start + (r ? L - 1 - e2 : e2);
            acc += row[x2] * (hn - H[e2 - e - 1]);
        }
    }
    double sum = block_sum_1024(acc, s_w);
    if (threadIdx.x == 0) out[0] = sum;
}

__global__ __launch_bounds__(1024) void k_p2_insert_straddle(const double* __restrict__ M2, int64_t ld2,
                                                            const int32_t* __restrict__ pos2sel, int n_arr,
                                                            const int32_t* __restrict__ arr_pos, int L,
                                                            const double* __restrict__ H, double* __restrict__ D)
{
    extern __shared__ __attribute__((aligned(16))) unsigned char smem[];
    int32_t* p = reinterpret_cast<int32_t*>(smem);
    __shared__ double s_w[16];
    for (int q = threadIdx.x; q < n_arr; q += 1024) p[q] = pos2sel[q];
    __syncthreads();
    straddle_body(M2, ld2, p, n_arr, arr_pos, blockIdx.x, L, H, s_w, D + blockIdx.x);
}

__global__ __launch_bounds__(1024) void k_p2_insert_cross(const double* __restrict__ M2, int64_t ld2,
                                                         const int32_t* __restrict__ pos2sel, int n_arr,
                                                         const int32_t* __restrict__ arr_pos, int new_start, int L,
                                                         const double* __restrict__ H, double* __restrict__ cross)
{
    extern __shared__ __attribute__((aligned(16))) unsigned char smem[];
    int32_t* p = reinterpret_cast<int32_t*>(smem);
    __shared__ double s_w[16];
    for (int q = threadIdx.x; q < n_arr; q += 1024) p[q] = pos2sel[q];
    __syncthreads();
    cross_body(M2, ld2, p, n_arr, arr_pos, blockIdx.x >> 1, blockIdx.x & 1, new_start, L, H, s_w, cross + blockIdx.x);
}

void launch_p2_insert_delta(const double* M2, int64_t ld2, const int32_t* pos2sel, int n_arr, const int32_t* arr_pos,
                            int S, int new_start, int L, const double* H, int n_base_blocks, double* out, hipStream_t s)
{
    const size_t lds = perm_lds_bytes(n_arr);
    launch_p2_base_partial(M2, ld2, pos2sel, n_arr, H, n_arr + L, n_base_blocks, out, s);
    ensure_dynamic_lds(reinterpret_cast<const void*>(k_p2_insert_straddle), g_lds_straddle, lds);
    ensure_dynamic_lds(reinterpret_cast<const void*>(k_p2_insert_cross), g_lds_cross, lds);
    hipLaunchKernelGGL(k_p2_insert_straddle, dim3(S), dim3(1024), lds, s, M2, ld2, pos2sel, n_arr, arr_pos, L, H,
                       out + n_base_blocks);
    hipLaunchKernelGGL(k_p2_insert_cross, dim3(2 * (S + 1)), dim3(1024), lds, s, M2, ld2, pos2sel, n_arr, arr_pos, new_start,
                       L, H, out + n_base_blocks + S);
}

__global__ __launch_bounds__(256) void k_insb_base(const InsStep* __restrict__ steps, int n_base_blocks)
{
    extern __shared__ __attribute__((aligned(16))) unsigned char smem[];
    int32_t* p = reinterpret_cast<int32_t*>(smem);
    const InsStep& d = steps[blockIdx.y];
    if (!d.active || d.st->fail >= 0) return;
    for (int q = threadIdx.x; q < d.n_arr; q += 256) p[q] = d.pos_cur[q];
    __syncthreads();
    base_partial_body(d.M2, d.ld2, p, d.n_arr, d.H, d.n_arr + d.L, blockIdx.x, n_base_blocks, d.partial + blockIdx.x);
}

__global__ __launch_bounds__(256) void k_insb_fast(const InsStep* __restrict__ steps, int n_base_blocks, int n_row_blocks,
                                                   int n_cross_blocks)
{
    extern __shared__ __attribute__((aligned(16))) unsigned char smem[];
    __shared__ double s_w[4];
    const InsStep& d = steps[blockIdx.y];
    if (!d.active || d.st->fail >= 0) return;
    const int S = d.S, n_arr = d.n_arr, L = d.L;
    const int lane = threadIdx.x & 63, wave = threadIdx.x >> 6;
    const int32_t* __restrict__ p = d.pos_cur;
    const int32_t* __restrict__ arr_pos = d.packed_cur + S;
    const double* __restrict__ H = d.H;
    const int n_base_here = (int)gridDim.x - n_row_blocks - n_cross_blocks;
    const int bx = (int)blockIdx.x - n_base_here;
    if (bx < 0) {
        const int slab = blockIdx.x;
        int32_t* pl = reinterpret_cast<int32_t*>(smem);
        for (int q = threadIdx.x; q < n_arr; q += 256) pl[q] = p[q];
        __syncthreads();
        base_partial_body(d.M2, d.ld2, pl, n_arr, H, n_arr + L, slab, n_base_blocks, d.partial + slab);
        return;
    }
    if (bx < n_row_blocks) {
        const int u = bx * 4 + wave;
        if (u >= n_arr) return;
        int below = 0;
        for (int j = lane; j <= S; j += 64) below += arr_pos[j] <= u;
#pragma unroll
        for (int off = 32; off >= 1; off >>= 1) below += __shfl_xor(below, off, 64);
        const int g = below - 1;
        const int P0 = arr_pos[g], P1 = arr_pos[g + 1];
        const double* __restrict__ row = d.M2 + (int64_t)p[u] * d.ld2;
        double acc = 0.0;
#pragma unroll 4
        for (int pos = lane; pos < P0; pos += 64) {
            const int dd = u - pos;
            acc -= row[p[pos]] * (H[dd + L - 1] - H[dd - 1]);
        }
#pragma unroll 4
        for (int pos = P1 + lane; pos < n_arr; pos += 64) {
            const int dd = pos - u;
            acc += row[p[pos]] * (H[dd + L - 1] - H[dd - 1]);
        }
        acc = wave_sum_s(acc);
        if (lane == 0) d.partial[n_base_blocks + u] = acc;
        return;
    }
    const int c = bx - n_row_blocks;
    if (c >= 2 * (S + 1)) return;
    const int g = c >> 1, r = c & 1, P = arr_pos[g];
    const double hn = H[n_arr + L - 1];
    double acc = 0.0;
    for (int e = wave; e < L; e += 4) {
        const int xe = d.new_start + (r ? L - 1 - e : e);
        const double* __restrict__ row = d.M2 + (int64_t)xe * d.ld2;
#pragma unroll 4
        for (int q = lane; q < n_arr; q += 64) {
            const int dd = q < P ? (P + e - q) : (q + L - (P + e));
            acc += row[p[q]] * (hn - H[dd - 1]);
        }
        for (int e2 = e + 1 + lane; e2 < L; e2 += 64) {
            const int x2 = d.new_start + (r ? L - 1 - e2 : e2);
            acc += row[x2] * (hn - H[e2 - e - 1]);
        }
    }
    const double sum = block_sum_256(acc, s_w);
    if (threadIdx.x == 0) d.partial[n_base_blocks + n_arr + c] = sum;
}

void launch_insb_fast(const InsStep* steps, int n_chrom, int max_S, int max_n_arr, int n_base_blocks, hipStream_t s)
{
    const size_t lds = perm_lds_bytes(max_n_arr);
    const int n_row_blocks = (max_n_arr + 3) / 4, n_cross_blocks = 2 * (max_S + 1);
    static const bool split = getenv("HICMI_P2_INSB_SPLIT") != nullptr;
    if (split) {
        ensure_dynamic_lds(reinterpret_cast<const void*>(k_insb_base), g_lds_insb_base, lds);
        hipLaunchKernelGGL(k_insb_base, dim3(n_base_blocks, n_chrom), dim3(256), lds, s, steps, n_base_blocks);
    }
    ensure_dynamic_lds(reinterpret_cast<const void*>(k_insb_fast), g_lds_insb_fast, lds);
    hipLaunchKernelGGL(k_insb_fast, dim3(n_row_blocks + n_cross_blocks + (split ? 0 : n_base_blocks), n_chrom), dim3(256), lds, s,
                       steps, n_base_blocks, n_row_blocks, n_cross_blocks);
}

static constexpr int G_TILE = 2048;
static constexpr int G_TMAX = 8;

template <bool H_IN_LDS>
__global__ __launch_bounds__(256) void k_p2_window_G(const double* __restrict__ M2, int64_t ld2,
                                                     const int32_t* __restrict__ pos2sel, int n,
                                                     const WindowBatchEntry* __restrict__ wb,
                                                     const double* H, double* __restrict__ G_all)
{
    extern __shared__ __attribute__((aligned(16))) unsigned char smem_g[];
    __shared__ double vals[G_TILE];
    __shared__ double part[4][64];
    const WindowBatchEntry& we = wb[blockIdx.y];
    const int p0 = we.p0, m = we.m;
    const int x = blockIdx.x, tid = threadIdx.x, tl = tid & 63, seg = tid >> 6;
    if (x >= m) return;
    double* __restrict__ G = G_all + we.g_off;
    const double* __restrict__ row = M2 + (int64_t)pos2sel[p0 + x] * ld2;
    const double hn = H[n - 1];
    if (H_IN_LDS) {
        double* hl = reinterpret_cast<double*>(smem_g);
        for (int i = tid; i < n; i += 256) hl[i] = H[i];
        __syncthreads();
        H = hl;
    }
    const int n_out = n - m;
    for (int tbase = 0; tbase < m; tbase += 64 * G_TMAX) {
        double acc[G_TMAX];
#pragma unroll
        for (int i = 0; i < G_TMAX; i++) acc[i] = 0.0;
        for (int base = 0; base < n_out; base += G_TILE) {
            const int cnt = n_out - base < G_TILE ? n_out - base : G_TILE;
            __syncthreads();
            for (int e = tid; e < cnt; e += 256) {
                int qq = base + e;
                vals[e] = row[pos2sel[qq < p0 ? qq : qq + m]];
            }
            __syncthreads();
            const int e0 = (cnt * seg) >> 2, e1 = (cnt * (seg + 1)) >> 2;
#pragma unroll
            for (int i = 0; i < G_TMAX; i++) {
                const int t = tbase + i * 64 + tl;
                if (t < m) {
                    const int pt = p0 + t;
                    double a = acc[i];
                    for (int e = e0; e < e1; e++) {
                        int qq = base + e;
                        int d = qq < p0 ? pt - qq : qq + m - pt;
                        a += vals[e] * (hn - H[d - 1]);
                    }
                    acc[i] = a;
                }
            }
        }
#pragma unroll
        for (int i = 0; i < G_TMAX; i++) {
            __syncthreads();
            part[seg][tl] = acc[i];
            __syncthreads();
            const int t = tbase + i * 64 + tl;
            if (seg == 0 && t < m) G[(int64_t)x * m + t] = (part[0][tl] + part[1][tl]) + (part[2][tl] + part[3][tl]);
        }
    }
}

static constexpr int WD_PER_WAVE = 4;
template <int WD_WAVES, bool BLOCK_IN_LDS>
__global__ __launch_bounds__(WD_WAVES * 64) void k_p2_window_delta(const double* __restrict__ M2, int64_t ld2, int n, int k,
                                                         const WindowBatchEntry* __restrict__ wb,
                                                         const int8_t* __restrict__ orders,
                                                         const uint8_t* __restrict__ orients, int n_ori, int n_cand,
                                                         const double* __restrict__ H, const double* __restrict__ G_all,
                                                         double* __restrict__ delta_all,
                                                         const int32_t* __restrict__ pos2sel, int max_m)
{
    extern __shared__ __attribute__((aligned(16))) unsigned char smem[];
    __shared__ int s_start[8], s_len[8], s_off[8], s_rev[8];
    __shared__ int s_ord[WD_WAVES][8], s_ori[WD_WAVES][8], s_slot[WD_WAVES][9];
    const WindowBatchEntry& we = wb[blockIdx.y];
    const int m = we.m;
    const double* __restrict__ G = G_all + we.g_off;
    const int tid = threadIdx.x, lane = tid & 63, wave = tid >> 6;
    int32_t* useq = reinterpret_cast<int32_t*>(smem) + (int64_t)wave * 2 * m;
    int32_t* xseq = useq + m;
    double* wt = reinterpret_cast<double*>(smem + (((size_t)max_m * 2 * WD_WAVES * sizeof(int32_t) + 15) & ~(size_t)15));
    double* wblk = wt + max_m;
    if (tid < k) {
        s_start[tid] = we.w.start[tid]; s_len[tid] = we.w.len[tid]; s_off[tid] = we.w.off[tid]; s_rev[tid] = we.w.rev[tid];
    }
    if (BLOCK_IN_LDS) {
        const int32_t* __restrict__ wsel = pos2sel + we.p0;
        for (int e = tid; e < m * m; e += WD_WAVES * 64) {
            const int x = e / m, y = e - x * m;
            wblk[e] = M2[(int64_t)wsel[x] * ld2 + wsel[y]];
        }
    }
    const double hn = H[n - 1];
    for (int d = tid; d < m; d += WD_WAVES * 64) wt[d] = d ? hn - H[d - 1] : 0.0;
    const int mm = m * m, ds = 64 / m, dt = 64 - ds * m;
    for (int it = 0; it < WD_PER_WAVE; it++) {
        const int c = (blockIdx.x * WD_WAVES + wave) * WD_PER_WAVE + it;
        const bool live = c < n_cand;
        if (live && lane < k) {
            s_ord[wave][lane] = orders[(int64_t)(c / n_ori) * k + lane];
            s_ori[wave][lane] = orients[(int64_t)(c % n_ori) * k + lane];
        }
        __syncthreads();
        if (live && lane == 0) {
            int acc_len = 0;
            s_slot[wave][0] = 0;
            for (int j = 0; j < k; j++) { acc_len += s_len[s_ord[wave][j]]; s_slot[wave][j + 1] = acc_len; }
        }
        __syncthreads();
        if (live) {
            for (int t = lane; t < m; t += 64) {
                int j = 0;
                while (j + 1 < k && s_slot[wave][j + 1] <= t) j++;
                const int jj = s_ord[wave][j], len = s_len[jj];
                const int ep = t - s_slot[wave][j];
                const int e = s_ori[wave][j] ? len - 1 - ep : ep;
                useq[t] = s_start[jj] + e;
                xseq[t] = s_off[jj] + (s_rev[jj] ? len - 1 - e : e);
            }
        }
        __syncthreads();
        if (live) {
            double acc = 0.0;
            for (int t = lane; t < m; t += 64) acc += G[(int64_t)xseq[t] * m + t];
            int ps = lane / m, pt = lane - ps * m;
#pragma unroll 8
            for (int q = lane; q < mm; q += 64) {
                const double v = BLOCK_IN_LDS ? wblk[xseq[ps] * m + xseq[pt]] : M2[(int64_t)useq[ps] * ld2 + useq[pt]];
                acc += v * wt[pt > ps ? pt - ps : 0];
                const int npt = pt + dt;
                const bool carry = npt >= m;
                ps += ds + (carry ? 1 : 0);
                pt = carry ? npt - m : npt;
            }
            acc = wave_sum_s(acc);
            if (lane == 0) delta_all[(int64_t)blockIdx.y * n_cand + c] = acc;
        }
        __syncthreads();
    }
}

void launch_p2_window_batch(const double* M2, int64_t ld2, const int32_t* pos2sel, int n, int k,
                            const WindowBatchEntry* wb, int n_win, int max_m, const int8_t* orders, const uint8_t* orients,
                            int n_ord, int n_ori, const double* H, double* G_all, double* delta_all, hipStream_t s)
{
    if (n_win <= 0 || max_m <= 0) return;
// ... 29 lines not shown
```

### include/hicmi.h

```cpp
#ifndef HICMI_H
#define HICMI_H

#include <stdint.h>

#ifdef __cplusplus
extern "C" {
#endif

#define HICMI_ABI_VERSION 1

#define HICMI_OK            0
#define HICMI_EINVAL       -1
#define HICMI_EHIP         -2
#define HICMI_ENOMEM       -3
#define HICMI_ESTATE       -4
#define HICMI_EUNSUPPORTED -5

typedef struct hicmi_ctx hicmi_ctx;

int         hicmi_abi_version(void);
const char *hicmi_last_error(void);
int         hicmi_device_count(int *count);

int hicmi_create(int device, hicmi_ctx **out);
int hicmi_destroy(hicmi_ctx *ctx);
int hicmi_stream(hicmi_ctx *ctx, void **stream_out);
int hicmi_synchronize(hicmi_ctx *ctx);

int hicmi_set_contacts_host(hicmi_ctx *ctx, const double *contacts, int64_t n);
int hicmi_set_contacts_host_f32(hicmi_ctx *ctx, const float *contacts, int64_t n);
int hicmi_set_contacts_device(hicmi_ctx *ctx, const double *d_contacts, int64_t n, int64_t ld);
int hicmi_contacts_device(hicmi_ctx *ctx, void **d_contacts_out, int64_t *n_out, int64_t *ld_out);

int hicmi_load_hicpro_matrix(const char *path, const int64_t *bin_ids, int64_t n, double *out, int threads,
                             int64_t *edges_out);

int hicmi_row_sums(hicmi_ctx *ctx, double *np_sum, double *seq_sum);

int hicmi_set_row_shard(hicmi_ctx *ctx, int64_t first, int64_t stride);
int hicmi_set_row_sums(hicmi_ctx *ctx, const double *np_sum, const double *seq_sum);

int hicmi_compact(hicmi_ctx *ctx, const int32_t *keep, int64_t n_keep);

int hicmi_upgma(hicmi_ctx *ctx, double *Z_out, int32_t *leaves_out);

int hicmi_rank_matrix(hicmi_ctx *ctx, const int32_t *order);
int hicmi_presort_state(hicmi_ctx *ctx, int *state_out, int64_t *tied_rows_out);
int hicmi_get_rank_rows(hicmi_ctx *ctx, int64_t row0, int64_t nrows, int inverse, uint16_t *out);
int hicmi_get_similarity_row(hicmi_ctx *ctx, int64_t row, double *out);

int hicmi_cut_scan(hicmi_ctx *ctx, int64_t start, int64_t M, double psig, int32_t *x_out, uint8_t *sig_out);

int hicmi_filter_scan(hicmi_ctx *ctx, int64_t start, int64_t c, int64_t n_rows, int64_t M, double psig,
                      int32_t *x_out, uint8_t *sig_out);

int hicmi_first_pass_cuts(hicmi_ctx *ctx, int64_t min_size, int64_t stop_ind, double psig, int32_t *cuts_out,
                          int64_t cuts_cap, int64_t *n_cuts_out, int32_t *m_log_out, int64_t log_cap, int64_t *n_log_out);
int hicmi_filter_cuts(hicmi_ctx *ctx, const int32_t *cuts_in, int64_t n_in, double psig, int32_t *cuts_out,
                      int64_t cuts_cap, int64_t *n_out, int64_t *warned_out);

#define HICMI_SCAN_MAX_SETS 64
int hicmi_first_pass_cuts_multi(hicmi_ctx *ctx, int64_t n_sets, const int64_t *min_size, const int64_t *stop_ind, double psig,
                                int32_t *cuts_out, int64_t cuts_cap, int64_t *n_cuts_out, int32_t *m_log_out, int64_t log_cap,
                                int64_t *n_log_out);
int hicmi_filter_cuts_multi(hicmi_ctx *ctx, int64_t n_sets, const int64_t *cand_off, const int32_t *cuts_in, const double *psig,
                            int32_t *cuts_out, int64_t cuts_cap, int64_t *n_out, int64_t *warned_out);

double hicmi_hypergeom_sf(int64_t x, int64_t M, int64_t n, int64_t N);
int hicmi_hypergeom_decide(int64_t x, int64_t M, int64_t n, int64_t N, double psig);

int hicmi_label_linkage(const double *Zraw, int64_t n, double *Z_out);
int hicmi_leaf_order(const double *Z, int64_t n, int32_t *leaves_out);
int hicmi_selftest_division(hicmi_ctx *ctx, uint64_t seed, int64_t samples, uint64_t *mismatches_out);
int hicmi_get_raw_merges(hicmi_ctx *ctx, double *Zraw_out);
int hicmi_nnchain_stats(hicmi_ctx *ctx, double *out6);

int hicmi_p2_select(hicmi_ctx *ctx, const int32_t *sel, int64_t n);
int hicmi_p2_total(hicmi_ctx *ctx, double *total_out);
int hicmi_p2_score(hicmi_ctx *ctx, const int32_t *perms, int64_t n_cand, int64_t n_used, double total,
                   double *scores_out);
int hicmi_p2_score_exact(hicmi_ctx *ctx, const int32_t *perms, int64_t n_cand, int64_t n_used, double total,
                         double *scores_out);

int hicmi_p2_layout(hicmi_ctx *ctx, const int32_t *scaf_start, const int32_t *scaf_len, int64_t n_scaf);
int hicmi_p2_set_arrangement(hicmi_ctx *ctx, const int32_t *ids, const uint8_t *rev, int64_t S);
int hicmi_p2_arrangement_total(hicmi_ctx *ctx, double *total_out);
int hicmi_p2_arrangement_score(hicmi_ctx *ctx, double total, double *score_out);
int hicmi_p2_score_insertions(hicmi_ctx *ctx, int32_t new_id, double total, double *scores_out);
int hicmi_p2_window_tables(hicmi_ctx *ctx, int64_t k, const int8_t *orders, int64_t n_orders,
                           const uint8_t *orients, int64_t n_orients);
int hicmi_p2_score_window(hicmi_ctx *ctx, int64_t first, int64_t k, double *delta_out);

int hicmi_p2_decide_window(hicmi_ctx *ctx, int64_t first, int64_t k, double total, double floor, double cur_fast,
                           int64_t *pick_out, double *best_out, double *pick_fast_out);
int hicmi_p2_window_shortlist(hicmi_ctx *ctx, int64_t first, int64_t count, int64_t k, double total, double floor,
                              double cur_fast, int64_t cap, int64_t *n_near_out, int64_t *idx_out, double *fast_out);
int hicmi_p2_decide_insertion(hicmi_ctx *ctx, const int32_t *ids, const uint8_t *rev, int64_t S, int32_t new_id,
                              int32_t new_rev_now, int64_t *gap_out, int32_t *rev_out, double *best_out);

int hicmi_p2_insert_all(hicmi_ctx *ctx, int32_t *ids, uint8_t *rev, int64_t S0, const int32_t *new_ids, int64_t n_new,
                        double *best_out);
int hicmi_p2_scan_pass(hicmi_ctx *ctx, int32_t *ids, uint8_t *rev, int64_t S, int64_t k, double total, double *best_io,
                       double *cur_fast_io, int32_t *improved_out);
int hicmi_p2_scan_all(hicmi_ctx *ctx, int32_t *ids, uint8_t *rev, int64_t S, int64_t k, double total, double *best_io,
                      double *cur_fast_io, int64_t *rounds_out);
int hicmi_p2_insert_all_multi(int64_t n_jobs, hicmi_ctx *const *ctxs, int32_t *const *ids, uint8_t *const *rev,
                              const int64_t *S0, const int32_t *const *new_ids, const int64_t *n_new, double *best_out);

int hicmi_p2_start_all(int64_t n_jobs, hicmi_ctx *const *ctxs, const int32_t *sel, const int64_t *n_sel,
                       const int32_t *scaf_start, const int32_t *scaf_len, const int64_t *n_scaf, const int32_t *first_ids,
                       const int64_t *k, const int8_t *const *orders, const int64_t *n_orders, const uint8_t *const *orients,
                       const int64_t *n_orients, double *total_out, int64_t *pick_out, double *cost_out, int32_t *status_out);
int hicmi_p2_scan_arranged(hicmi_ctx *ctx, int32_t *ids, uint8_t *rev, int64_t S, int64_t k, const int8_t *orders,
                           int64_t n_orders, const uint8_t *orients, int64_t n_orients, double *total_out, double *best_io,
                           int64_t *rounds_out);

int hicmi_p2_support(hicmi_ctx *ctx, const int32_t *ids, const uint8_t *rev, int64_t S, double total, double *scores_out,
                     int32_t *best_out);
int hicmi_p2_support_multi(int64_t n_jobs, hicmi_ctx *const *ctxs, const int32_t *const *ids, const uint8_t *const *rev,
                           const int64_t *S, const double *totals, double *const *scores_out, int32_t *const *best_out);

int hicmi_p2_breaks(hicmi_ctx *ctx, const int32_t *ids, const uint8_t *rev, int64_t S, double total, int64_t min_piece,
                    double *scores_out, int32_t *best_out);
int hicmi_p2_breaks_multi(int64_t n_jobs, hicmi_ctx *const *ctxs, const int32_t *const *ids, const uint8_t *const *rev,
                          const int64_t *S, const double *totals, int64_t min_piece, double *const *scores_out,
                          int32_t *const *best_out);

int hicmi_scan_valid_pairs(const char *path, const char *names_blob, const int64_t *name_off, int64_t n_names,
                           const int32_t *pair_a, const int32_t *pair_b, int64_t n_pairs, int threads,
                           int64_t *n_hits_out, int64_t *n_lines_out, void **handle_out);
int hicmi_scan_fetch(void *handle, int32_t *pair_idx, int64_t *pos1, int64_t *pos2);

int hicmi_plot_percentiles(hicmi_ctx *ctx, int kind, const int32_t *order, int64_t n_sel, const double *q, int64_t n_q,
                           double *out);
int hicmi_plot_downsample(hicmi_ctx *ctx, int kind, const int32_t *order, int64_t n_sel, int64_t px, double *out);

int hicmi_hmm_load_obs(hicmi_ctx *ctx, const int32_t *order, int64_t n, int64_t c, int64_t p);
int hicmi_hmm_set_obs(hicmi_ctx *ctx, const double *X, int64_t T, int64_t D);
int hicmi_hmm_set_width(hicmi_ctx *ctx, int64_t D);
int hicmi_hmm_get_obs(hicmi_ctx *ctx, int64_t row0, int64_t nrows, double *out);
int hicmi_hmm_dist2(hicmi_ctx *ctx, const int64_t *rows, int64_t k, double *out);
int hicmi_hmm_col_stats(hicmi_ctx *ctx, double *mean_out, double *m2_out);
int hicmi_hmm_kmeans(hicmi_ctx *ctx, const double *centers_in, int64_t max_iter, double tol, double *centers_out,
                     int32_t *labels_out, double *inertia_out, int64_t *n_iter_out);
int hicmi_hmm_fit(hicmi_ctx *ctx, const double *startprob, double *means, double *covars, double *transmat,
                  int64_t n_iter, double tol, double *logprob_out, int64_t *n_done_out);
int hicmi_hmm_decode(hicmi_ctx *ctx, const double *startprob, const double *means, const double *covars,
                     const double *transmat, int32_t *states_out);
#define HICMI_HMM_MAX_SLOTS 16
#define HICMI_HMM_MAX_PROBLEMS 256
int hicmi_hmm_load_obs_slot(hicmi_ctx *ctx, int64_t slot, const int32_t *order, int64_t n, int64_t c, int64_t p);
int hicmi_hmm_use_obs(hicmi_ctx *ctx, int64_t slot);
int hicmi_hmm_dist2_multi(hicmi_ctx *ctx, int64_t n_prob, const int64_t *slots, const int64_t *widths, const int64_t *nrows,
                          const int64_t *rows, double *out);
int hicmi_hmm_kmeans_multi(hicmi_ctx *ctx, int64_t n_prob, const int64_t *slots, const int64_t *widths, const int64_t *rows,
                           const int64_t *max_iter, const double *tol, double *centers_out, double *inertia_out,
                           int64_t *n_iter_out);

int hicmi_louvain_graph(hicmi_ctx *ctx, const int32_t *rows, int64_t m);
int hicmi_louvain_set_graph(hicmi_ctx *ctx, const double *A, int64_t m);
int hicmi_louvain_get_graph(hicmi_ctx *ctx, double *A_out, double *gdegrees_out, double *total_weight_out);
int hicmi_louvain_level0(hicmi_ctx *ctx, int64_t rounds, const uint64_t *states_in, int32_t *node2com_out,
                         uint64_t *states_out, int32_t *info_out, double *degrees_out, double *internals_out);
int hicmi_louvain_induced(hicmi_ctx *ctx, const int32_t *part, int64_t m, int64_t k, double *out);
int hicmi_louvain_modularity(hicmi_ctx *ctx, const int32_t *parts, int64_t rounds, int64_t m, double *q_out);

int hicmi_group_sums(hicmi_ctx *ctx, const int32_t *grp, const int32_t *scaf, int64_t n_groups, int64_t n_scaffolds,
                     double *bin_sums_out, double *scaffold_sums_out);

int hicmi_timing_reset(hicmi_ctx *ctx);
int hicmi_timing_enable(hicmi_ctx *ctx, int on);
int hicmi_timing_get(hicmi_ctx *ctx, char *names_out, int64_t names_cap, double *ms_out,
                     int64_t *launches_out, double *bytes_out, int64_t cap, int64_t *count_out);

#ifdef __cplusplus
}
#endif
#endif
```

Before: 124,800.

## Carry insertion base score across steps and fuse cost with apply kernel

```diff
diff --git a/hic_genome_assembler_amd/_lib.py b/hic_genome_assembler_amd/_lib.py
--- a/hic_genome_assembler_amd/_lib.py
+++ b/hic_genome_assembler_amd/_lib.py
@@ -74,6 +74,7 @@
     "hicmi_plot_percentiles": (ctypes.c_int, [_vp, ctypes.c_int, _vp, c_i64, _vp, c_i64, _vp]),
     "hicmi_plot_downsample": (ctypes.c_int, [_vp, ctypes.c_int, _vp, c_i64, c_i64, _vp]),
     "hicmi_p2_insert_all_multi": (ctypes.c_int, [c_i64, _vp, _vp, _vp, _vp, _vp, _vp, _vp]),
+    "hicmi_p2_insert_base_log": (ctypes.c_int, [_vp, _vp, c_i64, ctypes.POINTER(c_i64)]),
     "hicmi_p2_start_all": (ctypes.c_int, [c_i64] + [_vp] * 16),
     "hicmi_p2_scan_arranged": (ctypes.c_int, [_vp, _vp, _vp, c_i64, c_i64, _vp, c_i64, _vp, c_i64, ctypes.POINTER(c_dbl),
                                               ctypes.POINTER(c_dbl), ctypes.POINTER(c_i64)]),
@@ -498,6 +499,13 @@
         self._arr_sig = None
         return a, b, best.value
 
+    def p2_insert_base_log(self):
+        n = c_i64(0)
+        _check(self._lib.hicmi_p2_insert_base_log(self._h, None, 0, ctypes.byref(n)))
+        out = np.zeros(n.value, np.float64)
+        _check(self._lib.hicmi_p2_insert_base_log(self._h, _ptr(out), n.value, ctypes.byref(n)))
+        return out
+
     @staticmethod
     def p2_insert_all_multi(jobs):
         n = len(jobs)
diff --git a/hic_genome_assembler_amd/csrc/api.hip b/hic_genome_assembler_amd/csrc/api.hip
--- a/hic_genome_assembler_amd/csrc/api.hip
+++ b/hic_genome_assembler_amd/csrc/api.hip
@@ -119,6 +119,7 @@
     double* d_ins_partial = nullptr; int64_t ins_partial_cap = 0;
     unsigned char* d_ins_blob = nullptr; int64_t ins_blob_cap = 0;
     InsStep* d_ins_steps = nullptr; int64_t ins_steps_cap = 0;
+    std::vector<double> ins_base_log;
     SupRec* d_sup_recs = nullptr; int64_t sup_recs_cap = 0;
     BrkRec* d_brk_recs = nullptr; int64_t brk_recs_cap = 0;
     int32_t* d_gs_lists = nullptr; int64_t gs_lists_cap = 0;
@@ -2121,7 +2122,7 @@
         if (rc) return rc;
         rc = ensure(c->d_ins_T, c->ins_t_cap, (1 + 2 * (int64_t)INS_MAXC) * n_max);
         if (rc) return rc;
-        rc = ensure(c->d_ins_partial, c->ins_partial_cap, NB + n_max + 2 * (S_max + 1));
+        rc = ensure(c->d_ins_partial, c->ins_partial_cap, 2 * NB + n_max + 2 * (S_max + 1) + 1);
         if (rc) return rc;
         steps_max = std::max(steps_max, n_steps);
         blob_off[(size_t)j] = blob_bytes;
@@ -2135,6 +2136,7 @@
     std::vector<InsStep> table((size_t)(steps_max * nj));
     std::vector<int> max_n_used((size_t)steps_max, 0), max_S((size_t)steps_max, 0), max_n_arr((size_t)steps_max, 0);
     double algo = 0.0;
+    const bool split = insb_split();
     for (int j = 0; j < nj; j++) {
         InsJob& job = *jobs[(size_t)j];
         hicmi_ctx* c = job.c;
@@ -2159,12 +2161,13 @@
             d.T_total = c->d_ins_T; d.T_cand = c->d_ins_T + n_max; d.work = c->d_ins_T + (1 + (int64_t)INS_MAXC) * n_max;
             d.partial = c->d_ins_partial; d.log = log + t;
             d.n_arr = (int32_t)n_arr; d.S = (int32_t)(job.S + t); d.L = L; d.new_start = c->h_scaf_start[(size_t)nid];
-            d.new_id = nid; d.active = 1; d.step = (int32_t)t; d.last = t == n_steps - 1;
+            d.new_id = nid; d.active = 1; d.step = (int32_t)t; d.last = t == n_steps - 1; d.carry = split ? 0 : 1;
             max_n_used[(size_t)t] = std::max(max_n_used[(size_t)t], (int)(n_arr + L));
             max_S[(size_t)t] = std::max(max_S[(size_t)t], d.S);
             max_n_arr[(size_t)t] = std::max(max_n_arr[(size_t)t], (int)n_arr);
             const double nn = (double)n_arr, Ld = (double)L, sd = (double)d.S;
-            algo += 8.0 * (0.5 * nn * (nn - 1.0) + nn * nn + 2.0 * (sd + 1.0) * Ld * nn) + 4.0 * (nn + Ld) * (nn + Ld);
+            const double base_reads = (t == 0 || split) ? 0.5 * nn * (nn - 1.0) : 0.0;
+            algo += 8.0 * (base_reads + nn * nn + 2.0 * (sd + 1.0) * Ld * nn) + 4.0 * (nn + Ld) * (nn + Ld);
             n_arr += L;
         }
     }
@@ -2176,11 +2179,10 @@
         for (int64_t t = 0; t < steps_max; t++) {
             const InsStep* st_t = lead->d_ins_steps + t * nj;
             const int nu = max_n_used[(size_t)t];
-            launch_insb_fast(st_t, nj, max_S[(size_t)t], max_n_arr[(size_t)t], NB, lead->stream);
+            launch_insb_fast(st_t, nj, max_S[(size_t)t], max_n_arr[(size_t)t], NB, t == 0, lead->stream);
             launch_insb_shortlist(st_t, nj, max_S[(size_t)t], max_n_arr[(size_t)t], NB, kNearTop, max_c, lead->stream);
             launch_insb_diag_cand(st_t, nj, nu, lead->stream);
-            launch_insb_cost(st_t, nj, nu, lead->stream);
-            launch_insb_apply(st_t, nj, nu, lead->stream);
+            launch_insb_decide(st_t, nj, nu, NB, lead->stream);
         }
     }
     HIPCHK(hipGetLastError());
@@ -2214,6 +2216,8 @@
         const InsState* hst = reinterpret_cast<const InsState*>(blob.data() + blob_off[(size_t)j]);
         const InsLog* hlog = reinterpret_cast<const InsLog*>(blob.data() + blob_off[(size_t)j] + sizeof(InsState));
         const int64_t done = hst->fail >= 0 ? std::min<int64_t>(hst->fail, n_steps) : n_steps;
+        job.c->ins_base_log.resize((size_t)done);
+        for (int64_t t = 0; t < done; t++) job.c->ins_base_log[(size_t)t] = hlog[t].base;
         for (int64_t t = 0; t < done; t++) {
             if (hlog[t].gap < 0 || hlog[t].gap > job.S) return fail(HICMI_ESTATE, "insertion log out of range");
             apply_insertion(job.ids, job.rev, job.S, hlog[t].gap, job.new_ids[job.t + t], hlog[t].rev);
@@ -2258,6 +2262,7 @@
         int rc = check_insert_job(job, job.S);
         if (rc) return rc;
         if (job.S + job.n_new + 1 > 8192) job.device_ok = false;
+        job.c->ins_base_log.clear();
     }
     while (true) {
         std::vector<InsJob*> todo;
@@ -2290,6 +2295,15 @@
     int rc = run_insert_jobs(jobs);
     if (rc) return rc;
     *best_out = jobs[0].best;
+    return HICMI_OK;
+}
+
+int hicmi_p2_insert_base_log(hicmi_ctx* c, double* out, int64_t cap, int64_t* n_out)
+{
+    if (!c || !n_out || cap < 0 || (cap > 0 && !out)) return fail(HICMI_EINVAL, "bad arguments");
+    *n_out = (int64_t)c->ins_base_log.size();
+    const int64_t n = std::min<int64_t>(cap, *n_out);
+    for (int64_t t = 0; t < n; t++) out[t] = c->ins_base_log[(size_t)t];
     return HICMI_OK;
 }
 
diff --git a/hic_genome_assembler_amd/csrc/hicmi_internal.h b/hic_genome_assembler_amd/csrc/hicmi_internal.h
--- a/hic_genome_assembler_amd/csrc/hicmi_internal.h
+++ b/hic_genome_assembler_amd/csrc/hicmi_internal.h
@@ -287,12 +287,15 @@
 struct InsState {
     int32_t fail;
     int32_t n_short;
-    int32_t direct, pad;
+    int32_t direct;
+    int32_t have_base;
     int32_t gap[INS_MAXC], rev[INS_MAXC], idx[INS_MAXC];
     double total;
     double lit[INS_MAXC];
-};
-struct InsLog { int32_t gap, rev; double best; int32_t n_short, pad; };
+    double fast[INS_MAXC], fast0;
+    double base_score, base_mass;
+};
+struct InsLog { int32_t gap, rev; double best; int32_t n_short, pad; double base; };
 struct InsStep {
     const double* M2; const double* H; int64_t ld2;
     const int32_t* pos_cur; int32_t* pos_nxt;
@@ -300,14 +303,46 @@
     double *T_total, *T_cand, *work, *partial;
     InsState* st; InsLog* log;
     int32_t n_arr, S, L, new_start, new_id, active, step, last;
+    int32_t carry, pad;
 };
 void launch_insb_reset(const InsStep* steps, int n_chrom, hipStream_t s);
-void launch_insb_fast(const InsStep* steps, int n_chrom, int max_S, int max_n_arr, int n_base_blocks, hipStream_t s);
+bool insb_split();
+void launch_insb_fast(const InsStep* steps, int n_chrom, int max_S, int max_n_arr, int n_base_blocks, bool seed, hipStream_t s);
 void launch_insb_shortlist(const InsStep* steps, int n_chrom, int max_S, int max_n_arr, int n_base_blocks, double near_top,
                            int max_c, hipStream_t s);
 void launch_insb_diag_cand(const InsStep* steps, int n_chrom, int max_n_used, hipStream_t s);
-void launch_insb_cost(const InsStep* steps, int n_chrom, int max_n_used, hipStream_t s);
-void launch_insb_apply(const InsStep* steps, int n_chrom, int max_n_used, hipStream_t s);
+void launch_insb_decide(const InsStep* steps, int n_chrom, int max_n_used, int n_base_blocks, hipStream_t s);
+__device__ __forceinline__ void insb_apply_body(const InsStep& d, int gap, int rev)
+{
+    const int n_arr = d.n_arr, S = d.S, L = d.L, n_new = n_arr + L, S1 = S + 1;
+    const int32_t* __restrict__ id_in = d.packed_cur;
+    const int32_t* __restrict__ pos_in = d.packed_cur + S;
+    const int32_t* __restrict__ rev_in = d.packed_cur + 2 * S + 1;
+    int32_t* __restrict__ id_out = d.packed_nxt;
+    int32_t* __restrict__ pos_out = d.packed_nxt + S1;
+    int32_t* __restrict__ rev_out = d.packed_nxt + 2 * S1 + 1;
+    const int P = pos_in[gap];
+    for (int pos = threadIdx.x; pos < n_new; pos += 256) {
+        int v;
+        if (pos < P) v = d.pos_cur[pos];
+        else if (pos < P + L) v = d.new_start + (rev ? L - 1 - (pos - P) : pos - P);
+        else v = d.pos_cur[pos - L];
+        d.pos_nxt[pos] = v;
+    }
+    for (int j = threadIdx.x; j < S1; j += 256) {
+        id_out[j] = j < gap ? id_in[j] : (j == gap ? d.new_id : id_in[j - 1]);
+        rev_out[j] = j < gap ? rev_in[j] : (j == gap ? rev : rev_in[j - 1]);
+    }
+    for (int j = threadIdx.x; j <= S1; j += 256) pos_out[j] = j <= gap ? pos_in[j] : pos_in[j - 1] + L;
+}
+
+__device__ __forceinline__ void insb_carry(const InsStep& d, int n_base_blocks, double fast_applied)
+{
+    InsState* st = d.st;
+    st->base_score = fast_applied;
+    st->base_mass += d.partial[n_base_blocks + d.n_arr + 2 * (d.S + 1)];
+    st->have_base = d.carry;
+}
 
 static constexpr int SUP_BASE_SLABS = 64;
 static constexpr int SUP_MAX_S = 4096;
diff --git a/hic_genome_assembler_amd/csrc/k_part2.hip b/hic_genome_assembler_amd/csrc/k_part2.hip
--- a/hic_genome_assembler_amd/csrc/k_part2.hip
+++ b/hic_genome_assembler_amd/csrc/k_part2.hip
@@ -213,36 +213,41 @@
     hipLaunchKernelGGL(k_p2_cost_exact, dim3(n_cand), dim3(256), serial_lds_bytes(n_used), s, T, n_used, total, work, scores);
 }
 
+static constexpr int INSB_DIAG_GRID = 512;
+
 __global__ __launch_bounds__(64) void k_insb_diag_cand(const InsStep* __restrict__ steps, int sequential)
 {
     const InsStep& d = steps[blockIdx.y];
     if (!d.active || d.st->fail >= 0) return;
     const int ns = d.st->n_short;
     if (ns == 0) return;
-    const int n_used = d.n_arr + d.L, off = diag_of_block(blockIdx.x);
-    if (off >= n_used) return;
-    {
-        const IndexMap m = {d.pos_cur, d.n_arr, 0x3fffffff, d.new_start, 0};
-        const double acc = diag_sum_body(d.M2, d.ld2, m, n_used, off);
-        if (threadIdx.x == 0) d.T_total[off] = acc;
-    }
-    for (int q = 0; q < ns; q++) {
-        const IndexMap m = {d.pos_cur, d.packed_cur[d.S + d.st->gap[q]], d.L, d.new_start, d.st->rev[q]};
-        const double acc = sequential ? diag_sum_sequential(d.M2, d.ld2, m, n_used, off) : diag_sum_body(d.M2, d.ld2, m, n_used, off);
-        if (threadIdx.x == 0) d.T_cand[(int64_t)q * n_used + off] = acc;
-    }
-}
-
-__global__ __launch_bounds__(256) void k_insb_cost(const InsStep* __restrict__ steps)
+    const int n_used = d.n_arr + d.L, n_blocks = ((n_used - 1) + 63) & ~63;
+    for (int vb = blockIdx.x; vb < n_blocks; vb += gridDim.x) {
+        const int off = diag_of_block(vb);
+        if (off >= n_used) continue;
+        __syncthreads();
+        {
+            const IndexMap m = {d.pos_cur, d.n_arr, 0x3fffffff, d.new_start, 0};
+            const double acc = diag_sum_body(d.M2, d.ld2, m, n_used, off);
+            if (threadIdx.x == 0) d.T_total[off] = acc;
+        }
+        for (int q = 0; q < ns; q++) {
+            const IndexMap m = {d.pos_cur, d.packed_cur[d.S + d.st->gap[q]], d.L, d.new_start, d.st->rev[q]};
+            const double acc = sequential ? diag_sum_sequential(d.M2, d.ld2, m, n_used, off) : diag_sum_body(d.M2, d.ld2, m, n_used, off);
+            if (threadIdx.x == 0) d.T_cand[(int64_t)q * n_used + off] = acc;
+        }
+    }
+}
+
+__global__ __launch_bounds__(256) void k_insb_decide(const InsStep* __restrict__ steps, int n_base_blocks)
 {
     extern __shared__ __attribute__((aligned(16))) unsigned char smem_ic[];
-    __shared__ double s_total;
-    const InsStep& d = steps[blockIdx.y];
-    if (!d.active || d.st->fail >= 0) return;
-    const int cand = blockIdx.x;
-    if (cand >= d.st->n_short) return;
-    const int n_used = d.n_arr + d.L;
-    {
+    __shared__ double s_total, s_lit[INS_MAXC];
+    const InsStep& d = steps[blockIdx.x];
+    InsState* st = d.st;
+    if (!d.active || st->fail >= 0 || st->direct) return;
+    const int ns = st->n_short, n_used = d.n_arr + d.L;
+    if (ns > 0) {
         double* t = reinterpret_cast<double*>(smem_ic);
         const bool staged = n_used <= SERIAL_LDS_MAX;
         if (staged) {
@@ -254,24 +259,38 @@
             if (staged) acc = serial_sum_lds(t, 1, n_used, 0.0);
             else for (int i = 1; i < n_used; i++) acc += d.T_total[i];
             s_total = acc;
-            if (cand == 0) d.st->total = acc;
-        }
-        __syncthreads();
-    }
-    cost_exact_body(d.T_cand + (int64_t)cand * n_used, n_used, s_total, d.work + (int64_t)cand * n_used, d.st->lit + cand);
+            st->total = acc;
+        }
+        __syncthreads();
+        for (int q = 0; q < ns; q++) {
+            cost_exact_body(d.T_cand + (int64_t)q * n_used, n_used, s_total, d.work + (int64_t)q * n_used, s_lit + q);
+            __syncthreads();
+        }
+    }
+    double best = 0.0;
+    int pick = -1;
+    for (int q = 0; q < ns; q++) if (s_lit[q] > best) { best = s_lit[q]; pick = q; }
+    const int gap = pick >= 0 ? st->gap[pick] : 0, rev = pick >= 0 ? st->rev[pick] : 0;
+    insb_apply_body(d, gap, rev);
+    if (threadIdx.x == 0) {
+        for (int q = 0; q < ns; q++) st->lit[q] = s_lit[q];
+        d.log->gap = gap; d.log->rev = rev; d.log->best = pick >= 0 ? best : 0.0; d.log->n_short = ns;
+        insb_carry(d, n_base_blocks, pick >= 0 ? st->fast[pick] : st->fast0);
+    }
 }
 
 void launch_insb_diag_cand(const InsStep* steps, int n_chrom, int max_n_used, hipStream_t s)
 {
     if (max_n_used < 2) return;
-    hipLaunchKernelGGL(k_insb_diag_cand, dim3(diag_grid(max_n_used), n_chrom), dim3(64), 0, s, steps, numba_trace_order() ? 1 : 0);
-}
-
-void launch_insb_cost(const InsStep* steps, int n_chrom, int max_n_used, hipStream_t s)
-{
-    ensure_dynamic_lds(reinterpret_cast<const void*>(k_insb_cost), g_lds_insb_cost, 65536);
+    const int grid = diag_grid(max_n_used) < INSB_DIAG_GRID ? diag_grid(max_n_used) : INSB_DIAG_GRID;
+    hipLaunchKernelGGL(k_insb_diag_cand, dim3(grid, n_chrom), dim3(64), 0, s, steps, numba_trace_order() ? 1 : 0);
+}
+
+void launch_insb_decide(const InsStep* steps, int n_chrom, int max_n_used, int n_base_blocks, hipStream_t s)
+{
+    ensure_dynamic_lds(reinterpret_cast<const void*>(k_insb_decide), g_lds_insb_cost, 65536);
     const int max_staged = max_n_used < SERIAL_LDS_MAX ? max_n_used : SERIAL_LDS_MAX;
-    hipLaunchKernelGGL(k_insb_cost, dim3(INS_MAXC, n_chrom), dim3(256), serial_lds_bytes(max_staged), s, steps);
+    hipLaunchKernelGGL(k_insb_decide, dim3(n_chrom), dim3(256), serial_lds_bytes(max_staged), s, steps, n_base_blocks);
 }
 
 __global__ __launch_bounds__(256) void k_p2_score(const double* __restrict__ M2, int64_t ld2,
diff --git a/hic_genome_assembler_amd/csrc/k_part2_insert.hip b/hic_genome_assembler_amd/csrc/k_part2_insert.hip
--- a/hic_genome_assembler_amd/csrc/k_part2_insert.hip
+++ b/hic_genome_assembler_amd/csrc/k_part2_insert.hip
@@ -5,7 +5,7 @@
 __global__ void k_insb_reset(const InsStep* __restrict__ steps)
 {
     InsState* st = steps[blockIdx.x].st;
-    if (threadIdx.x == 0 && steps[blockIdx.x].active) { st->fail = -1; st->n_short = 0; st->direct = 0; }
+    if (threadIdx.x == 0 && steps[blockIdx.x].active) { st->fail = -1; st->n_short = 0; st->direct = 0; st->have_base = 0; st->base_score = 0.0; st->base_mass = 0.0; }
 }
 
 void launch_insb_reset(const InsStep* steps, int n_chrom, hipStream_t s)
@@ -22,8 +22,8 @@
 {
     extern __shared__ __attribute__((aligned(16))) unsigned char smem_sl[];
     double* buf = reinterpret_cast<double*>(smem_sl);
-    __shared__ double s_base, s_wmax[SL_THREADS / 64];
-    __shared__ int s_any[SL_THREADS / 64], s_cnt, s_list[SL_LIST];
+    __shared__ double s_base, s_mass, s_wmax[SL_THREADS / 64];
+    __shared__ int s_any[SL_THREADS / 64], s_cnt, s_list[SL_LIST], s_take[3];
     const InsStep& d = steps[blockIdx.x];
     InsState* st = d.st;
     const int tid = threadIdx.x;
@@ -33,9 +33,10 @@
     const int32_t* __restrict__ arr_pos = d.packed_cur + S;
     double* part = buf + S + 1;
     const bool staged = n_arr <= SL_STAGE_MAX;
+    const bool carried = d.carry && st->have_base;
     const int n_stage = n_base_blocks + (staged ? n_arr : 0);
-    for (int i = tid; i < n_stage; i += SL_THREADS) part[i] = partial[i];
-    if (tid == 0) s_cnt = 0;
+    for (int i = (carried ? n_base_blocks : 0) + tid; i < n_stage; i += SL_THREADS) part[i] = partial[i];
+    if (tid == 0) { s_cnt = 0; s_take[0] = 0; }
     __syncthreads();
     for (int g = tid; g < S; g += SL_THREADS) {
         const int P0 = arr_pos[g], P1 = arr_pos[g + 1];
@@ -44,14 +45,29 @@
         else for (int u = P0; u < P1; u++) acc += partial[n_base_blocks + u];
         buf[g + 1] = acc;
     }
+    if (!carried && d.carry && tid >= SL_THREADS - 64) {
+        const double* __restrict__ mslab = partial + n_base_blocks + n_arr + 2 * (S + 1) + 1;
+        double m = 0.0;
+        for (int i = tid - (SL_THREADS - 64); i < n_base_blocks; i += 64) m += mslab[i];
+        m = wave_sum_s(m);
+        if (tid == SL_THREADS - 64) s_mass = m;
+    }
     __syncthreads();
     if (tid == 0) {
-        s_base = serial_sum_lds(part, 0, n_base_blocks, 0.0);
+        if (carried) s_base = st->base_score + (d.H[n_arr + d.L - 1] - d.H[n_arr - 1]) * st->base_mass;
+        else {
+            s_base = serial_sum_lds(part, 0, n_base_blocks, 0.0);
+            if (d.carry) st->base_mass = s_mass;
+        }
         buf[0] = 0.0;
         serial_prefix_lds(buf, 1, S + 1, 0.0);
     }
     __syncthreads();
     const double base = s_base;
+    if (carried && !isfinite(base)) {
+        if (tid == 0) { st->fail = d.step; st->n_short = 0; st->direct = 0; }
+        return;
+    }
     const double* __restrict__ cross = partial + n_base_blocks + n_arr;
     const int n_cand = 2 * (S + 1);
     auto fast_of = [&](int i) -> double {
@@ -59,6 +75,7 @@
         const int r = (i & 1) ? (first ^ 1) : first;
         return base - buf[g] + cross[2 * g + r];
     };
+    if (tid == 0) { d.log->base = base; st->fast0 = fast_of(0); }
     double mx = -__builtin_inf();
     int any = 0;
     for (int i = tid; i < n_cand; i += SL_THREADS) {
@@ -93,29 +110,45 @@
     if (tid == 0) {
         int cnt = s_cnt;
         st->direct = 0;
-        if (cnt > max_c && !(d.L == 1 && cnt <= 2 * max_c && cnt <= SL_LIST)) { st->fail = d.step; st->n_short = 0; return; }
-        for (int a = 1; a < cnt; a++) {
-            const int v = s_list[a];
-            int b = a - 1;
-            while (b >= 0 && s_list[b] > v) { s_list[b + 1] = s_list[b]; b--; }
-            s_list[b + 1] = v;
+        bool declined = cnt > max_c && !(d.L == 1 && cnt <= 2 * max_c && cnt <= SL_LIST);
+        if (!declined) {
+            for (int a = 1; a < cnt; a++) {
+                const int v = s_list[a];
+                int b = a - 1;
+                while (b >= 0 && s_list[b] > v) { s_list[b + 1] = s_list[b]; b--; }
+                s_list[b + 1] = v;
+            }
+            if (d.L == 1) {
+                int w = 0;
+                for (int q = 0; q < cnt; q++) {
+                    const int i = s_list[q];
+                    if ((i & 1) && w > 0 && s_list[w - 1] == i - 1) continue;
+                    s_list[w++] = i;
+                }
+                cnt = w;
+                declined = cnt > max_c;
+            }
         }
-        if (d.L == 1) {
-            int w = 0;
+        if (declined) { st->fail = d.step; st->n_short = 0; }
+        else {
             for (int q = 0; q < cnt; q++) {
-                const int i = s_list[q];
-                if ((i & 1) && w > 0 && s_list[w - 1] == i - 1) continue;
-                s_list[w++] = i;
+                const int i = s_list[q], g = i >> 1, first = g & 1;
+                st->idx[q] = i; st->gap[q] = g; st->rev[q] = (i & 1) ? (first ^ 1) : first; st->fast[q] = fast_of(i);
             }
-            cnt = w;
-            if (cnt > max_c) { st->fail = d.step; st->n_short = 0; return; }
+            if (cnt == 1 && !d.last && top > 0.0) {
+                st->direct = 1; st->n_short = 0;
+                s_take[0] = 1; s_take[1] = st->gap[0]; s_take[2] = st->rev[0];
+            }
+            else st->n_short = cnt;
         }
-        for (int q = 0; q < cnt; q++) {
-            const int i = s_list[q], g = i >> 1, first = g & 1;
-            st->idx[q] = i; st->gap[q] = g; st->rev[q] = (i & 1) ? (first ^ 1) : first;
-        }
-        if (cnt == 1 && !d.last && top > 0.0) { st->direct = 1; st->n_short = 0; }
-        else st->n_short = cnt;
+    }
+    __syncthreads();
+    if (!s_take[0]) return;
+    const int gap = s_take[1], rev = s_take[2];
+    insb_apply_body(d, gap, rev);
+    if (tid == 0) {
+        d.log->gap = gap; d.log->rev = rev; d.log->best = __builtin_nan(""); d.log->n_short = -1;
+        insb_carry(d, n_base_blocks, st->fast[0]);
     }
 }
 
@@ -131,48 +164,4 @@
                        max_c < 1 ? 1 : (max_c > INS_MAXC ? INS_MAXC : max_c));
 }
 
-__global__ __launch_bounds__(256) void k_insb_apply(const InsStep* __restrict__ steps)
-{
-    const InsStep& d = steps[blockIdx.y];
-    const InsState* __restrict__ st = d.st;
-    if (!d.active || st->fail >= 0) return;
-    const int n_arr = d.n_arr, S = d.S, L = d.L, n_new = n_arr + L;
-    if ((int)blockIdx.x * 256 >= n_new && blockIdx.x != 0) return;
-    double best = 0.0;
-    int pick = -1;
-    const int ns = st->n_short, direct = st->direct;
-    for (int q = 0; q < ns; q++) if (st->lit[q] > best) { best = st->lit[q]; pick = q; }
-    if (direct) { pick = 0; best = __builtin_nan(""); }
-    const int gap = pick >= 0 ? st->gap[pick] : 0, rev = pick >= 0 ? st->rev[pick] : 0;
-    const int32_t* __restrict__ id_in = d.packed_cur;
-    const int32_t* __restrict__ pos_in = d.packed_cur + S;
-    const int32_t* __restrict__ rev_in = d.packed_cur + 2 * S + 1;
-    const int P = pos_in[gap];
-    const int pos = blockIdx.x * 256 + threadIdx.x;
-    if (pos < n_new) {
-        int v;
-        if (pos < P) v = d.pos_cur[pos];
-        else if (pos < P + L) v = d.new_start + (rev ? L - 1 - (pos - P) : pos - P);
-        else v = d.pos_cur[pos - L];
-        d.pos_nxt[pos] = v;
-    }
-    if (blockIdx.x == 0) {
-        const int S1 = S + 1;
-        int32_t* __restrict__ id_out = d.packed_nxt;
-        int32_t* __restrict__ pos_out = d.packed_nxt + S1;
-        int32_t* __restrict__ rev_out = d.packed_nxt + 2 * S1 + 1;
-        for (int j = threadIdx.x; j < S1; j += 256) {
-            id_out[j] = j < gap ? id_in[j] : (j == gap ? d.new_id : id_in[j - 1]);
-            rev_out[j] = j < gap ? rev_in[j] : (j == gap ? rev : rev_in[j - 1]);
-        }
-        for (int j = threadIdx.x; j <= S1; j += 256) pos_out[j] = j <= gap ? pos_in[j] : pos_in[j - 1] + L;
-        if (threadIdx.x == 0) { d.log->gap = gap; d.log->rev = rev; d.log->best = pick >= 0 ? best : 0.0; d.log->n_short = direct ? -1 : ns; }
-    }
 }
-
-void launch_insb_apply(const InsStep* steps, int n_chrom, int max_n_used, hipStream_t s)
-{
-    hipLaunchKernelGGL(k_insb_apply, dim3((max_n_used + 255) / 256, n_chrom), dim3(256), 0, s, steps);
-}
-
-}
diff --git a/hic_genome_assembler_amd/csrc/k_part2_search.hip b/hic_genome_assembler_amd/csrc/k_part2_search.hip
--- a/hic_genome_assembler_amd/csrc/k_part2_search.hip
+++ b/hic_genome_assembler_amd/csrc/k_part2_search.hip
@@ -163,11 +163,32 @@
     base_partial_body(d.M2, d.ld2, p, d.n_arr, d.H, d.n_arr + d.L, blockIdx.x, n_base_blocks, d.partial + blockIdx.x);
 }
 
+__device__ __forceinline__ void base_mass_partial_body(const double* __restrict__ M2, int64_t ld2, const int32_t* p, int n_arr,
+                                                       const double* __restrict__ H, int n_tot, int blk, int n_blk,
+                                                       double* __restrict__ out_base, double* __restrict__ out_mass)
+{
+    __shared__ double s_wb[4], s_wm[4];
+    const int lane = threadIdx.x & 63, wave = threadIdx.x >> 6;
+    const double hn = H[n_tot - 1];
+    double acc = 0.0, mass = 0.0;
+    for (int a = blk * 4 + wave; a < n_arr - 1; a += n_blk * 4) {
+        const double* __restrict__ row = M2 + (int64_t)p[a] * ld2;
+#pragma unroll 4
+        for (int b = a + 1 + lane; b < n_arr; b += 64) {
+            const double v = row[p[b]];
+            acc += v * (hn - H[b - a - 1]);
+            mass += v;
+        }
+    }
+    const double sum = block_sum_256(acc, s_wb), msum = block_sum_256(mass, s_wm);
+    if (threadIdx.x == 0) { out_base[0] = sum; out_mass[0] = msum; }
+}
+
 __global__ __launch_bounds__(256) void k_insb_fast(const InsStep* __restrict__ steps, int n_base_blocks, int n_row_blocks,
                                                    int n_cross_blocks)
 {
     extern __shared__ __attribute__((aligned(16))) unsigned char smem[];
-    __shared__ double s_w[4];
+    __shared__ double s_w[4], s_w2[4];
     const InsStep& d = steps[blockIdx.y];
     if (!d.active || d.st->fail >= 0) return;
     const int S = d.S, n_arr = d.n_arr, L = d.L;
@@ -182,7 +203,8 @@
         int32_t* pl = reinterpret_cast<int32_t*>(smem);
         for (int q = threadIdx.x; q < n_arr; q += 256) pl[q] = p[q];
         __syncthreads();
-        base_partial_body(d.M2, d.ld2, pl, n_arr, H, n_arr + L, slab, n_base_blocks, d.partial + slab);
+        base_mass_partial_body(d.M2, d.ld2, pl, n_arr, H, n_arr + L, slab, n_base_blocks, d.partial + slab,
+                               d.partial + n_base_blocks + n_arr + 2 * (S + 1) + 1 + slab);
         return;
     }
     if (bx < n_row_blocks) {
@@ -214,35 +236,50 @@
     if (c >= 2 * (S + 1)) return;
     const int g = c >> 1, r = c & 1, P = arr_pos[g];
     const double hn = H[n_arr + L - 1];
-    double acc = 0.0;
+    double acc = 0.0, mass = 0.0;
     for (int e = wave; e < L; e += 4) {
         const int xe = d.new_start + (r ? L - 1 - e : e);
         const double* __restrict__ row = d.M2 + (int64_t)xe * d.ld2;
 #pragma unroll 4
         for (int q = lane; q < n_arr; q += 64) {
             const int dd = q < P ? (P + e - q) : (q + L - (P + e));
-            acc += row[p[q]] * (hn - H[dd - 1]);
+            const double v = row[p[q]];
+            acc += v * (hn - H[dd - 1]);
+            mass += v;
         }
         for (int e2 = e + 1 + lane; e2 < L; e2 += 64) {
             const int x2 = d.new_start + (r ? L - 1 - e2 : e2);
-            acc += row[x2] * (hn - H[e2 - e - 1]);
+            const double v = row[x2];
+            acc += v * (hn - H[e2 - e - 1]);
+            mass += v;
         }
     }
     const double sum = block_sum_256(acc, s_w);
     if (threadIdx.x == 0) d.partial[n_base_blocks + n_arr + c] = sum;
-}
-
-void launch_insb_fast(const InsStep* steps, int n_chrom, int max_S, int max_n_arr, int n_base_blocks, hipStream_t s)
-{
-    const size_t lds = perm_lds_bytes(max_n_arr);
+    if (c == 0) {
+        const double msum = block_sum_256(mass, s_w2);
+        if (threadIdx.x == 0) d.partial[n_base_blocks + n_arr + 2 * (S + 1)] = msum;
+    }
+}
+
+bool insb_split()
+{
+    static const bool split = getenv("HICMI_P2_INSB_SPLIT") != nullptr;
+    return split;
+}
+
+void launch_insb_fast(const InsStep* steps, int n_chrom, int max_S, int max_n_arr, int n_base_blocks, bool seed, hipStream_t s)
+{
     const int n_row_blocks = (max_n_arr + 3) / 4, n_cross_blocks = 2 * (max_S + 1);
-    static const bool split = getenv("HICMI_P2_INSB_SPLIT") != nullptr;
-    if (split) {
+    if (insb_split()) {
+        const size_t lds = perm_lds_bytes(max_n_arr);
         ensure_dynamic_lds(reinterpret_cast<const void*>(k_insb_base), g_lds_insb_base, lds);
         hipLaunchKernelGGL(k_insb_base, dim3(n_base_blocks, n_chrom), dim3(256), lds, s, steps, n_base_blocks);
-    }
-    ensure_dynamic_lds(reinterpret_cast<const void*>(k_insb_fast), g_lds_insb_fast, lds);
-    hipLaunchKernelGGL(k_insb_fast, dim3(n_row_blocks + n_cross_blocks + (split ? 0 : n_base_blocks), n_chrom), dim3(256), lds, s,
+        seed = false;
+    }
+    const size_t lds = seed ? perm_lds_bytes(max_n_arr) : 0;
+    if (seed) ensure_dynamic_lds(reinterpret_cast<const void*>(k_insb_fast), g_lds_insb_fast, lds);
+    hipLaunchKernelGGL(k_insb_fast, dim3(n_row_blocks + n_cross_blocks + (seed ? n_base_blocks : 0), n_chrom), dim3(256), lds, s,
                        steps, n_base_blocks, n_row_blocks, n_cross_blocks);
 }
 
diff --git a/include/hicmi.h b/include/hicmi.h
--- a/include/hicmi.h
+++ b/include/hicmi.h
@@ -107,6 +107,8 @@
 int hicmi_p2_insert_all_multi(int64_t n_jobs, hicmi_ctx *const *ctxs, int32_t *const *ids, uint8_t *const *rev,
                               const int64_t *S0, const int32_t *const *new_ids, const int64_t *n_new, double *best_out);
 
+int hicmi_p2_insert_base_log(hicmi_ctx *ctx, double *out, int64_t cap, int64_t *n_out);
+
 int hicmi_p2_start_all(int64_t n_jobs, hicmi_ctx *const *ctxs, const int32_t *sel, const int64_t *n_sel,
                        const int32_t *scaf_start, const int32_t *scaf_len, const int64_t *n_scaf, const int32_t *first_ids,
                        const int64_t *k, const int8_t *const *orders, const int64_t *n_orders, const uint8_t *const *orients,
```

Result: slower. 123,500 (-1.0%).
